# Apokleos/kata-xpu-device-plugin

Hardware: AMD Instinct MI355X
Metric: Allocate() p50 latency (lower is better)
Workload: dtype n/a; 1 GPU; model=kata-xpu-device-plugin-amd pod-churn, node=8x MI355X (mock sysfs, vfio-pci), gpus_per_pod=1, discovered_gpus=8, concurrent_clients=1, parallelism=1 churn client(s), one plugin daemon

## Files before the change

kata_xpu_device_plugin_amd/plugin/manager.py:

```python
from __future__ import annotations

import os
import signal
import threading
from typing import Dict, List, Optional

from ..cdi.spec import build_spec, write_spec
from ..config import Config
from ..discovery.naming import resource_name
from ..discovery.sysfs import NodeInventory, XPUDevice, scan_node
from ..health.watcher import NodeWatcher
from ..topology.hive import GPUTopology, load_topology
from ..utils.log import configure as configure_logging, get_logger
from .server import XPUDevicePlugin
from .state import DeviceState

log = get_logger(__name__)


class PluginManager:
    def __init__(self, cfg: Config):
        cfg.validate()
        self.cfg = cfg
        self.inventory: Optional[NodeInventory] = None
        self.topology: Optional[GPUTopology] = None
        self.plugins: Dict[str, XPUDevicePlugin] = {}
        self.states: Dict[str, DeviceState] = {}
        self.watcher: Optional[NodeWatcher] = None
        self.cdi_spec_path: Optional[str] = None
        self._stop = threading.Event()
        self._register = True
        self._rescan_lock = threading.Lock()
        self._metrics = None
        self._amdsmi = None
        self._gpu_probe = None
        self._rescan_thread = None

    def _group_by_resource(self, inv: NodeInventory) -> Dict[str, Dict[str, XPUDevice]]:
        out: Dict[str, Dict[str, XPUDevice]] = {}
        for gid, dev in inv.devices.items():
            rname = resource_name(
                dev.model_device_id,
                namespace=self.cfg.resource_namespace,
                pci_ids_paths=tuple(self.cfg.pci_ids_paths),
                is_vf=dev.is_vf,
                unified=self.cfg.unified_resource_name,
            )
            out.setdefault(rname, {})[gid] = dev
        return out

    def _write_cdi(self, inv: NodeInventory) -> Optional[str]:
        if not inv.devices:
            from ..cdi.spec import spec_path
            for fmt in ("yaml", "json"):
                stale = spec_path(self.cfg.cdi_dir, self.cfg.cdi_spec_name, fmt)
                if os.path.exists(stale):
                    try:
                        os.unlink(stale)
                    except OSError:
                        pass
            log.info("no devices: no CDI spec written")
            return None
        spec = build_spec(inv, self.cfg.cdi_kind, self.cfg.dev_root,
                          self.cfg.cdi_version)
        return write_spec(
            spec, self.cfg.cdi_dir, self.cfg.cdi_spec_name, self.cfg.cdi_format
        )

    def setup(self) -> None:
        inv = scan_node(self.cfg)
        self.inventory = inv
        log.info(
            "discovered %d xPU device(s) in %.1f ms (%d %s function(s) total)",
            len(inv.devices), inv.scan_wall_s * 1e3, len(inv.all_functions),
            "/".join(f"{v:04x}" for v in self.cfg.vendor_allowlist),
        )
        self.topology = load_topology(self.cfg, inv)
        log.info("xGMI topology source: %s (%d hive-mapped GPUs)",
                 self.topology.source, len(self.topology.hive_of))

        self.cdi_spec_path = self._write_cdi(inv)

        for rname, devs in sorted(self._group_by_resource(inv).items()):
            state = DeviceState(devs)
            self.states[rname] = state
            self.plugins[rname] = XPUDevicePlugin(
                self.cfg, rname, state, self.topology
            )
            log.info("resource %s: %d device(s): %s", rname, len(devs),
                     ",".join(sorted(devs)))

    def start(self, register: bool = True) -> None:
        self._register = register
        if not self.plugins:
            log.warning("no devices discovered; serving nothing (will still "
                        "watch for kubelet restarts)")
        for plugin in self.plugins.values():
            plugin.start(register=register)
        self.watcher = NodeWatcher(
            self.cfg,
            self.states,
            on_socket_removed=self._on_socket_removed,
            on_kubelet_restarted=self._on_kubelet_restarted,
            plugin_socket_names={p.socket_name for p in self.plugins.values()},
            on_cdi_spec_removed=self._on_cdi_spec_removed,
            cdi_spec_names={os.path.basename(self.cdi_spec_path)}
            if self.cdi_spec_path else set(),
        )
        self.watcher.start()
        self.watcher.wait_ready()
        if self.cfg.amdsmi_health:
            from ..health.amdsmi_health import AmdSmiPoller
            self._amdsmi = AmdSmiPoller(
                self.cfg.health_poll_interval_s, self._on_amdsmi_health,
                on_xgmi=self._on_xgmi_telemetry,
            )
            self._amdsmi.start()
        if self.cfg.gpu_probe_interval_s > 0:
            from ..health.probe_poller import GpuProbePoller
            self._gpu_probe = GpuProbePoller(
                self.cfg.gpu_probe_interval_s, self._on_probe_health
            )
            self._gpu_probe.start()
        if self.cfg.rescan_interval_s > 0:
            self._rescan_thread = threading.Thread(
                target=self._rescan_loop, name="kxdp-rescan", daemon=True)
            self._rescan_thread.start()
        if self.cfg.metrics_port:
            from ..metrics import MetricsExporter
            self._metrics = MetricsExporter(self)
            self._metrics.start(self.cfg.metrics_port)
        if self.cfg.gc_tuning:
            self._tune_gc()
        if self.cfg.cpu_affinity:
            self._pin_cpus(self.cfg.cpu_affinity)

    @staticmethod
    def _pin_cpus(spec: str) -> None:
        cpus = set()
        try:
            for part in spec.split(","):
                part = part.strip()
                if not part:
                    continue
                if "-" in part:
                    lo, hi = part.split("-", 1)
                    cpus.update(range(int(lo), int(hi) + 1))
                else:
                    cpus.add(int(part))
            if cpus:
                os.sched_setaffinity(0, cpus)
                log.info("pinned daemon to CPUs %s", sorted(cpus))
        except (ValueError, OSError) as e:
            log.warning("cpu_affinity %r not applied: %s", spec, e)

    @staticmethod
    def _tune_gc() -> None:
        import gc
        gc.collect()
        gc.freeze()
        gc.set_threshold(50_000, 20, 20)

    def _on_socket_removed(self, socket_name: str) -> None:
        for plugin in list(self.plugins.values()):
            if plugin.socket_name == socket_name and not self._stop.is_set():
                if plugin.consume_expected_removal():
                    log.info("socket removal of %s was self-inflicted; skipping", socket_name)
                    continue
                if os.path.exists(plugin.socket_path) and plugin.serving:
                    continue
                try:
                    log.warning("EXTERNAL socket removal; restarting %s", plugin.resource_name)
                    plugin.restart()
                except Exception:
                    log.exception("restart of %s failed", plugin.resource_name)

    def _on_cdi_spec_removed(self, name: str) -> None:
        if self._stop.is_set() or self.inventory is None:
            return
        try:
            self.cdi_spec_path = self._write_cdi(self.inventory)
        except Exception:
            log.exception("CDI spec regeneration failed")

    def _on_amdsmi_health(self, bdf: str, healthy: bool, reasons) -> None:
        for state in list(self.states.values()):
            for gid in state.device_ids():
                dev = state.device(gid)
                if dev and bdf in (fn.bdf.lower() for fn in dev.functions):
                    if not healthy:
                        log.warning("amd-smi: %s unhealthy: %s", bdf, reasons)
                    state.set_health(gid, healthy, source="amdsmi")
                    return

    def _on_xgmi_telemetry(self, snap) -> None:
        if self.topology is None:
            return
        sick = {bdf for bdf, dh in snap.items() if dh.xgmi_sick}
        if sick != set(self.topology.degraded):
            if sick:
                log.warning("xGMI degraded link(s) on %s — excluded from "
                            "hive placement", sorted(sick))
            else:
                log.info("xGMI links recovered; hive placement restored")
            self.topology.set_degraded(sick)

    def _rescan_loop(self) -> None:
        while not self._stop.wait(self.cfg.rescan_interval_s):
            try:
                self.rescan()
            except Exception:
                log.exception("periodic rescan failed")

    def _on_probe_health(self, bdf: str, healthy: bool) -> None:
        bdf = bdf.lower()
        for state in list(self.states.values()):
            for gid in state.device_ids():
                dev = state.device(gid)
                if dev and bdf in (fn.bdf.lower() for fn in dev.functions):
                    if not healthy:
                        log.warning("gpu probe: %s unhealthy", bdf)
                    state.set_health(gid, healthy, source="probe")
                    return

    def _on_kubelet_restarted(self) -> None:
        if self._stop.is_set():
            return
        for plugin in list(self.plugins.values()):
            try:
                plugin.register_with_kubelet()
            except Exception:
                log.exception("re-registration of %s failed", plugin.resource_name)

    def install_signal_handlers(self) -> None:
        def _sig(signum, frame):
            log.info("signal %d — shutting down", signum)
            self._stop.set()

        def _hup(signum, frame):
            log.info("SIGHUP — rescanning inventory")
            threading.Thread(target=self._safe_rescan, name="kxdp-hup-rescan",
                             daemon=True).start()

        signal.signal(signal.SIGTERM, _sig)
        signal.signal(signal.SIGINT, _sig)
        signal.signal(signal.SIGHUP, _hup)

    def _safe_rescan(self) -> None:
        try:
            if not self._stop.is_set():
                self.rescan()
        except Exception:
            log.exception("SIGHUP rescan failed")

    def run_forever(self) -> None:
        self.install_signal_handlers()
        self._stop.wait()
        self.stop()

    def stop(self) -> None:
        self._stop.set()
        if self.watcher is not None:
            self.watcher.stop()
            self.watcher = None
        if self._amdsmi is not None:
            self._amdsmi.stop()
            self._amdsmi = None
        if self._gpu_probe is not None:
            self._gpu_probe.stop()
            self._gpu_probe = None
        for plugin in list(self.plugins.values()):
            plugin.stop()
        if self._metrics is not None:
            self._metrics.stop()
            self._metrics = None

    @staticmethod
    def _inventory_signature(inv: NodeInventory):
        return {
            gid: (tuple(dev.bdfs), dev.model_device_id, dev.numa_node,
                  dev.is_vf)
            for gid, dev in inv.devices.items()
        }

    def rescan(self) -> bool:
        with self._rescan_lock:
            return self._rescan_locked()

    def _rescan_locked(self) -> bool:
        inv = scan_node(self.cfg)
        if self.inventory is not None and \
                self._inventory_signature(inv) == \
                self._inventory_signature(self.inventory):
            return False
        log.info("rescan: inventory changed (%d → %d devices)",
                 len(self.inventory.devices) if self.inventory else 0,
                 len(inv.devices))
        self.inventory = inv
        prev_degraded = self.topology.degraded if self.topology else frozenset()
        self.topology = load_topology(self.cfg, inv)
        self.topology.degraded = prev_degraded
        self.cdi_spec_path = self._write_cdi(inv)
        grouped = self._group_by_resource(inv)

        for rname, state in list(self.states.items()):
            if rname in grouped:
                state.replace_devices(grouped[rname])
                self.plugins[rname].topo = self.topology

        retiring = [r for r in self.plugins if r not in grouped]
        if retiring and self.watcher is not None:
            self.watcher.plugin_socket_names = {
                p.socket_name for r, p in self.plugins.items()
                if r not in retiring}
        for rname in retiring:
            plugin = self.plugins.pop(rname)
            self.states.pop(rname, None)
            try:
                plugin.stop()
            except Exception:
                log.exception("stopping retired plugin %s failed", rname)
            log.info("resource %s retired (no devices after rescan)", rname)

        for rname in sorted(set(grouped) - set(self.plugins)):
            state = DeviceState(grouped[rname])
            plugin = XPUDevicePlugin(self.cfg, rname, state, self.topology)
            self.states[rname] = state
            self.plugins[rname] = plugin
            if self.watcher is not None:
                try:
                    plugin.start(register=self._register)
                    log.info("resource %s: started dynamically (%d devices)",
                             rname, len(grouped[rname]))
                except Exception:
                    log.exception("dynamic start of %s failed", rname)

        if self.watcher is not None:
            self.watcher.plugin_socket_names = {
                p.socket_name for p in self.plugins.values()}
        return True


def main(argv: Optional[List[str]] = None) -> int:
    import argparse

    parser = argparse.ArgumentParser(
        prog="kata-xpu-device-plugin-amd",
        description="MI355X-native Kubernetes device plugin for VFIO/Kata GPU passthrough",
    )
    Config.add_args(parser)
    args = parser.parse_args(argv)
    cfg = Config.from_args(args)
    configure_logging(cfg.log_level)
    mgr = PluginManager(cfg)
    mgr.install_signal_handlers()
    mgr.setup()
    mgr.start()
    mgr.run_forever()
    return 0


if __name__ == "__main__":
    raise SystemExit(main())
```

kata_xpu_device_plugin_amd/plugin/server.py:

```python
from __future__ import annotations

import asyncio
import atexit
import os
import threading
import time
import weakref
from typing import Dict, List, Optional

import grpc
import grpc.aio

from ..cdi.spec import ANNOTATION_PREFIX, qualified_name
from ..config import Config, STRATEGY_CDI_ANNOTATIONS, STRATEGY_CDI_CRI
from ..discovery.sysfs import read_hex, read_link_base
from ..topology.hive import GPUTopology, preferred_sets
from ..utils.log import get_logger
from . import api
from .state import DeviceState

log = get_logger(__name__)

try:
    from .. import _native as _NATIVE
except ImportError:
    _NATIVE = None

ENV_CDI_VENDOR_CLASS = "KUBERNETES_CDI_VENDOR_CLASS"
ENV_PCI_RESOURCE_PREFIX = "PCI_RESOURCE_"

_DEVICE_PLUGIN_PATH = "/v1beta1.DevicePlugin/"

_LIVE_NATIVE = weakref.WeakSet()


@atexit.register
def _stop_native_servers() -> None:
    for plugin in list(_LIVE_NATIVE):
        srv = plugin._native_server
        if srv is not None:
            try:
                srv.stop(0.0)
            except Exception:
                pass


def _stream_open() -> None:
    """DeviceState subscription of one open native ListAndWatch stream."""


def native_server_available() -> bool:
    return _NATIVE is not None and hasattr(_NATIVE, "GrpcServer")


class AllocationError(Exception):
    pass


class XPUDevicePlugin:

    def __init__(
        self,
        cfg: Config,
        resource_name: str,
        state: DeviceState,
        topo: GPUTopology,
        socket_name: Optional[str] = None,
    ):
        self.cfg = cfg
        self.resource_name = resource_name
        self.state = state
        self.topo = topo
        short = resource_name.split("/", 1)[1].lower()
        self.socket_name = socket_name or f"{cfg.plugin_socket_prefix}-{short}.sock"
        self.socket_path = os.path.join(cfg.kubelet_socket_dir, self.socket_name)
        self._aio_server: Optional[grpc.aio.Server] = None
        self._loop: Optional[asyncio.AbstractEventLoop] = None
        self._thread: Optional[threading.Thread] = None
        self._stop = threading.Event()
        self._serving = threading.Event()
        self._lifecycle = threading.Lock()
        self._removal_lock = threading.Lock()
        self._expected_removals = 0
        self.watcher_servicer = None
        self.watcher_socket_path: Optional[str] = None
        self._allocations = 0
        self._allocate_failures = 0
        self._last_allocate_s = 0.0
        self._allocate_seconds_total = 0.0
        self._native_server = None
        self._native_unsubscribe = None
        self._stream_subscriptions: List = []
        self._devices_dir = os.path.join(cfg.sysfs_root, "bus", "pci", "devices")
        self._vendor_list = list(cfg.vendor_allowlist)
        self._qn_cache: Dict[str, str] = {}
        self._bdf_cache = None
        self._timing = {"allocate_us": [], "preferred_us": [],
                        "loop_lag_us": []} if cfg.rpc_timing_path else None
        self._env_res_name = ENV_PCI_RESOURCE_PREFIX + resource_name.upper(
        ).replace("/", "_").replace(".", "_").replace("-", "_")

    def _native_stats(self):
        srv = self._native_server
        return srv.stats() if srv is not None else (0, 0, None, 0.0)

    @property
    def allocations(self) -> int:
        return self._allocations + self._native_stats()[0]

    @allocations.setter
    def allocations(self, v: int) -> None:
        self._allocations = v

    @property
    def allocate_failures(self) -> int:
        return self._allocate_failures + self._native_stats()[1]

    @allocate_failures.setter
    def allocate_failures(self, v: int) -> None:
        self._allocate_failures = v

    @property
    def last_allocate_s(self) -> float:
        last = self._native_stats()[2]
        return self._last_allocate_s if not last else last

    @last_allocate_s.setter
    def last_allocate_s(self, v: float) -> None:
        self._last_allocate_s = v

    @property
    def allocate_seconds_total(self) -> float:
        return self._allocate_seconds_total + self._native_stats()[3]

    @allocate_seconds_total.setter
    def allocate_seconds_total(self, v: float) -> None:
        self._allocate_seconds_total = v

    def _qn(self, gid: str) -> str:
        qn = self._qn_cache.get(gid)
        if qn is None:
            qn = self._qn_cache[gid] = qualified_name(self.cfg.cdi_kind, gid)
        return qn

    async def GetDevicePluginOptions(self, request, context):
        return api.DevicePluginOptions(
            pre_start_required=False,
            get_preferred_allocation_available=True,
        )

    def _device_list(self, snapshot=None) -> List[object]:
        devs = []
        if snapshot is None:
            snapshot = self.state.snapshot()
        for dev, healthy in snapshot:
            d = api.Device(
                id=dev.id,
                health=api.HEALTHY if healthy else api.UNHEALTHY,
            )
            if dev.numa_node >= 0:
                d.topology.nodes.add(id=dev.numa_node)
            devs.append(d)
        return devs

    async def ListAndWatch(self, request, context):
        loop = asyncio.get_running_loop()
        event = asyncio.Event()

        def _notify() -> None:
            try:
                loop.call_soon_threadsafe(event.set)
            except RuntimeError:
                pass

        unsubscribe = self.state.subscribe(_notify)
        try:
            yield api.ListAndWatchResponse(devices=self._device_list())
            while not self._stop.is_set():
                await event.wait()
                event.clear()
                if self._stop.is_set():
                    break
                yield api.ListAndWatchResponse(devices=self._device_list())
        finally:
            unsubscribe()

    def _revalidate_many(self, ids: List[str]) -> None:
        groups = []
        for gid in ids:
            dev = self.state.device(gid)
            if dev is None:
                raise AllocationError(f"unknown device id {gid}")
            if self.cfg.reject_unhealthy and not self.state.is_healthy(gid):
                raise AllocationError(f"device {gid} is Unhealthy")
            groups.append((gid, [fn.bdf for fn in dev.functions]))
        if self.cfg.native != "off":
            if _NATIVE is None and self.cfg.native == "require":
                raise RuntimeError("_native extension required but missing")
            if _NATIVE is not None:
                err = _NATIVE.revalidate_groups(
                    self._devices_dir, groups,
                    self._vendor_list, self.cfg.required_driver,
                )
                if err:
                    raise AllocationError(err)
                return
        for gid, _bdfs in groups:
            self._revalidate_py(gid)

    def _revalidate_py(self, gid: str) -> None:
        dev = self.state.device(gid)
        assert dev is not None
        devices_dir = self._devices_dir
        for fn in dev.functions:
            p = os.path.join(devices_dir, fn.bdf)
            if read_link_base(os.path.join(p, "iommu_group")) != gid:
                raise AllocationError(f"device {fn.bdf} no longer in IOMMU group {gid}")
            vendor = read_hex(os.path.join(p, "vendor"))
            if vendor not in set(self.cfg.vendor_allowlist):
                raise AllocationError(f"device {fn.bdf} vendor {vendor:#x} not allowed")
            if read_link_base(os.path.join(p, "driver")) != self.cfg.required_driver:
                raise AllocationError(
                    f"device {fn.bdf} not bound to {self.cfg.required_driver}"
                )

    def _container_response(self, ids: List[str]):
        resp = api.ContainerAllocateResponse()
        strategy = self.cfg.device_list_strategy
        bdfs: List[str] = []
        if ids and strategy not in (STRATEGY_CDI_CRI, STRATEGY_CDI_ANNOTATIONS):
            vfio_ctl = os.path.join(self.cfg.dev_root, "vfio", "vfio")
            resp.devices.add(
                container_path=vfio_ctl, host_path=vfio_ctl, permissions="rw"
            )
        for gid in ids:
            dev = self.state.device(gid)
            assert dev is not None
            bdfs.extend(dev.bdfs)
            if strategy == STRATEGY_CDI_CRI:
                resp.cdi_devices.add(name=self._qn(gid))
            elif strategy == STRATEGY_CDI_ANNOTATIONS:
                key = f"{ANNOTATION_PREFIX}vfio{gid}"
                resp.annotations[key] = self._qn(gid)
            else:
                path = os.path.join(self.cfg.dev_root, dev.vfio_node)
                resp.devices.add(
                    container_path=path, host_path=path, permissions="rw"
                )
        if strategy in (STRATEGY_CDI_CRI, STRATEGY_CDI_ANNOTATIONS):
            resp.envs[ENV_CDI_VENDOR_CLASS] = self.cfg.cdi_kind
        resp.envs[self._env_res_name] = ",".join(bdfs)
        return resp

    async def Allocate(self, request, context):
        t0 = time.perf_counter()
        response = api.AllocateResponse()
        try:
            for creq in request.container_requests:
                ids = list(creq.devices_ids)
                self._revalidate_many(ids)
                response.container_responses.append(self._container_response(ids))
        except AllocationError as e:
            self.allocate_failures += 1
            log.warning("Allocate(%s) rejected: %s", self.resource_name, e)
            await context.abort(grpc.StatusCode.INVALID_ARGUMENT, str(e))
        self.allocations += 1
        self.last_allocate_s = time.perf_counter() - t0
        self.allocate_seconds_total += self.last_allocate_s
        if self._timing is not None:
            self._timing["allocate_us"].append(self.last_allocate_s * 1e6)
        return response

    async def GetPreferredAllocation(self, request, context):
        return self._preferred_allocation(request)

    def _preferred_allocation(self, request):
        t0 = time.perf_counter() if self._timing is not None else 0.0
        resp = api.PreferredAllocationResponse()
        gen = self.state.generation
        cached = self._bdf_cache
        if cached is not None and cached[0] == gen:
            bdf_of = cached[1]
        else:
            bdf_of = self.state.bdf_map()
            self._bdf_cache = (gen, bdf_of)
        for creq in request.container_requests:
            available = [d for d in creq.available_device_ids if d in bdf_of]
            must = list(creq.must_include_device_ids)
            pick = preferred_sets(
                self.topo, bdf_of, available, must, creq.allocation_size
            )
            resp.container_responses.add(device_ids=pick)
        if self._timing is not None:
            self._timing["preferred_us"].append(
                (time.perf_counter() - t0) * 1e6)
        return resp

    async def PreStartContainer(self, request, context):
        return api.PreStartContainerResponse()

    def start(self, register: bool = True) -> None:
        with self._lifecycle:
            self._start_locked(register)

    def _use_native_server(self) -> bool:
        want = self.cfg.grpc_server
        if want == "aio":
            return False
        if native_server_available() and self.cfg.native != "off":
            return True
        if want == "native":
            raise RuntimeError(
                "grpc_server=native needs the _native extension "
                "(and native != off)")
        if self.cfg.native == "require":
            raise RuntimeError("_native extension required but missing")
        return False

    def _start_locked(self, register: bool) -> None:
        self._stop.clear()
        if self._use_native_server():
            self._start_native()
        else:
            self._start_aio()
        ch = grpc.insecure_channel(f"unix://{self.socket_path}")
        try:
            grpc.channel_ready_future(ch).result(timeout=self.cfg.grpc_timeout_s)
        finally:
            ch.close()
        self._serving.set()
        if register and self.cfg.registration_mode in ("legacy", "both"):
            try:
                self.register_with_kubelet()
            except Exception as e:
                log.warning("kubelet registration failed (%s); serving "
                            "anyway and retrying in background", e)
                self._spawn_registration_retry()
        log.info("plugin %s serving on %s (%s registration)",
                 self.resource_name, self.socket_path,
                 self.cfg.registration_mode)

    def _start_aio(self) -> None:
        self._loop_ready = threading.Event()
        self._start_error: Optional[BaseException] = None
        self._thread = threading.Thread(
            target=self._serve_thread,
            name=f"kxdp-grpc-{self.resource_name.split('/')[-1]}",
            daemon=True,
        )
        self._thread.start()
        if not self._loop_ready.wait(self.cfg.grpc_timeout_s):
            raise RuntimeError(f"gRPC server for {self.resource_name} "
                               "did not start in time")
        if self._start_error is not None:
            self._thread.join(timeout=2.0)
            raise self._start_error

    def _start_native(self) -> None:
        os.makedirs(self.cfg.kubelet_socket_dir, exist_ok=True)
        if os.path.exists(self.socket_path):
            self._note_expected_removal()
            os.unlink(self.socket_path)
        paths = [self.socket_path]
        if self.cfg.registration_mode in ("watcher", "both"):
            from .watcher_registration import (
                SERVICE_PATH_PREFIX,
                WatcherRegistrationServicer,
            )
            os.makedirs(self.cfg.plugins_registry_dir, exist_ok=True)
            self.watcher_servicer = WatcherRegistrationServicer(
                self.resource_name, self.socket_path)
            self.watcher_socket_path = os.path.join(
                self.cfg.plugins_registry_dir, self.socket_name)
            if os.path.exists(self.watcher_socket_path):
                os.unlink(self.watcher_socket_path)
            paths.append(self.watcher_socket_path)
        srv = _NATIVE.GrpcServer(paths)
        p = _DEVICE_PLUGIN_PATH
        srv.register_constant(
            p + "GetDevicePluginOptions",
            api.DevicePluginOptions(
                pre_start_required=False,
                get_preferred_allocation_available=True,
            ).SerializeToString())
        srv.register_constant(
            p + "PreStartContainer",
            api.PreStartContainerResponse().SerializeToString())
        srv.register_watch(p + "ListAndWatch", self._on_watch_streams)
        srv.register_unary(p + "GetPreferredAllocation",
                           self._preferred_allocation_bytes)
        srv.configure_allocate(
            p + "Allocate",
            strategy=self.cfg.device_list_strategy,
            reject_unhealthy=bool(self.cfg.reject_unhealthy),
            cdi_kind=self.cfg.cdi_kind,
            env_name=self._env_res_name,
            dev_root=self.cfg.dev_root,
            devices_dir=self._devices_dir,
            vendors=self._vendor_list,
            required_driver=self.cfg.required_driver,
            on_reject=self._log_rejection,
            timing=self._timing is not None,
        )
        if self.watcher_servicer is not None and len(paths) > 1:
            srv.register_unary(SERVICE_PATH_PREFIX + "GetInfo",
                               self.watcher_servicer.get_info_bytes)
            srv.register_unary(
                SERVICE_PATH_PREFIX + "NotifyRegistrationStatus",
                self.watcher_servicer.notify_registration_status_bytes)
        self._native_server = srv
        self._native_unsubscribe = self.state.subscribe_snapshot(
            self._push_native_state)
        try:
            srv.start()
        except BaseException:
            self._native_unsubscribe()
            self._native_unsubscribe = None
            self._native_server = None
            raise
        _LIVE_NATIVE.add(self)

    def _push_native_state(self, snapshot, generation) -> None:
        srv = self._native_server
        if srv is None:
            return
        dev_root = self.cfg.dev_root
        rows = []
        for dev, healthy in snapshot:
            qn = self._qn(dev.id)
            rows.append((
                dev.id,
                [fn.bdf for fn in dev.functions],
                bool(healthy),
                api.CDIDevice(name=qn).SerializeToString(),
                f"{ANNOTATION_PREFIX}vfio{dev.id}",
                qn,
                os.path.join(dev_root, dev.vfio_node),
            ))
        srv.update_table(rows)
        srv.publish(api.ListAndWatchResponse(
            devices=self._device_list(snapshot)).SerializeToString())

    def _on_watch_streams(self, delta: int) -> None:
        subs = self._stream_subscriptions
        for _ in range(delta):
            subs.append(self.state.subscribe(_stream_open))
        for _ in range(-delta):
            if subs:
                subs.pop()()

    def _preferred_allocation_bytes(self, request: bytes) -> bytes:
        return self._preferred_allocation(
            api.PreferredAllocationRequest.FromString(request)
        ).SerializeToString()

    def _log_rejection(self, err: str) -> None:
        log.warning("Allocate(%s) rejected: %s", self.resource_name, err)

    def _stop_native(self) -> None:
        srv = self._native_server
        if srv is None:
            return
        if self._native_unsubscribe is not None:
            self._native_unsubscribe()
            self._native_unsubscribe = None
        srv.stop(1.0)
        n, fails, last, total = srv.stats()
        if self._timing is not None:
            self._timing["allocate_us"] = list(srv.allocate_timing_us())
            self._timing["loop_lag_us"] = []
            self._dump_timing()
        self._native_server = None
        _LIVE_NATIVE.discard(self)
        while self._stream_subscriptions:
            self._stream_subscriptions.pop()()
        self._allocations += n
        self._allocate_failures += fails
        self._allocate_seconds_total += total
        if last:
            self._last_allocate_s = last

    def _spawn_registration_retry(self) -> None:
        def retry():
            delay = 1.0
            while self._serving.is_set() and not self._stop.is_set():
                if self._stop.wait(delay):
                    return
                if not self._serving.is_set():
                    return
                try:
                    self.register_with_kubelet()
                    log.info("kubelet registration succeeded after retry")
                    return
                except Exception:
                    delay = min(delay * 2, 30.0)

        threading.Thread(target=retry, daemon=True,
                         name=f"kxdp-register-retry-{self.socket_name}").start()

    def _serve_thread(self) -> None:
        loop = asyncio.new_event_loop()
        self._loop = loop
        asyncio.set_event_loop(loop)

        async def _main():
            server = grpc.aio.server(
                options=[("grpc.max_concurrent_streams", 64),
                         ("grpc.optimization_target", "latency")])
            api.add_device_plugin_servicer(server, self)
            os.makedirs(self.cfg.kubelet_socket_dir, exist_ok=True)
            if os.path.exists(self.socket_path):
                self._note_expected_removal()
                os.unlink(self.socket_path)
            server.add_insecure_port(f"unix://{self.socket_path}")
            if self.cfg.registration_mode in ("watcher", "both"):
                from .watcher_registration import (
                    WatcherRegistrationServicer,
                    add_watcher_registration_servicer,
                )
                os.makedirs(self.cfg.plugins_registry_dir, exist_ok=True)
                self.watcher_servicer = WatcherRegistrationServicer(
                    self.resource_name, self.socket_path)
                self.watcher_socket_path = os.path.join(
                    self.cfg.plugins_registry_dir, self.socket_name)
                add_watcher_registration_servicer(server, self.watcher_servicer)
                if os.path.exists(self.watcher_socket_path):
                    os.unlink(self.watcher_socket_path)
                server.add_insecure_port(f"unix://{self.watcher_socket_path}")
            await server.start()
            self._aio_server = server
            self._stop_async = asyncio.Event()
            lag_task = None
            if self._timing is not None:
                async def _lag_monitor():
                    while not self._stop_async.is_set():
                        t0 = time.perf_counter()
                        await asyncio.sleep(0.001)
                        lag = (time.perf_counter() - t0 - 0.001) * 1e6
                        self._timing["loop_lag_us"].append(max(0.0, lag))
                        if len(self._timing["loop_lag_us"]) > 200_000:
                            del self._timing["loop_lag_us"][:100_000]
                lag_task = asyncio.ensure_future(_lag_monitor())
            self._loop_ready.set()
            await self._stop_async.wait()
            if lag_task is not None:
                lag_task.cancel()
            await server.stop(grace=1.0)
            if self._timing is not None:
                self._dump_timing()

        try:
            loop.run_until_complete(_main())
        except BaseException as e:
            self._start_error = e
            self._loop_ready.set()
        finally:
            try:
                loop.close()
            except Exception:
                pass

    def _dump_timing(self) -> None:
        import json
        import statistics as stats

        def dist(xs):
            if not xs:
                return None
            xs = sorted(xs)
            n = len(xs)
            return {"n": n,
                    "p50": round(xs[n // 2], 1),
                    "p90": round(xs[min(n - 1, int(n * 0.9))], 1),
                    "p99": round(xs[min(n - 1, int(n * 0.99))], 1),
                    "max": round(xs[-1], 1),
                    "mean": round(stats.fmean(xs), 1)}

        out = {k: dist(v) for k, v in self._timing.items()}
        path = f"{self.cfg.rpc_timing_path}.{self.socket_name}.json"
        try:
            with open(path, "w") as f:
                json.dump(out, f, indent=1)
            log.info("rpc timing breakdown → %s", path)
        except OSError as e:
            log.warning("could not write rpc timing: %s", e)

    def register_with_kubelet(self) -> None:
        ch = grpc.insecure_channel(f"unix://{self.cfg.kubelet_socket}")
        try:
            grpc.channel_ready_future(ch).result(timeout=self.cfg.grpc_timeout_s)
            stub = api.RegistrationStub(ch)
            stub.Register(
                api.RegisterRequest(
                    version=api.VERSION,
                    endpoint=self.socket_name,
                    resource_name=self.resource_name,
                    options=api.DevicePluginOptions(
                        pre_start_required=False,
                        get_preferred_allocation_available=True,
                    ),
                ),
                timeout=self.cfg.grpc_timeout_s,
            )
        finally:
            ch.close()

    def stop(self) -> None:
        with self._lifecycle:
            self._stop_locked()

    def _stop_locked(self) -> None:
        self._stop.set()
        self._serving.clear()
        self.state.poke()
        if os.path.exists(self.socket_path):
            self._note_expected_removal()
        self._stop_native()
        if self._loop is not None and getattr(self, "_stop_async", None) is not None:
            try:
                self._loop.call_soon_threadsafe(self._stop_async.set)
            except RuntimeError:
                pass
        if self._thread is not None:
            self._thread.join(timeout=5.0)
            self._thread = None
        self._aio_server = None
        self._loop = None
        for path in (self.socket_path,
                     getattr(self, "watcher_socket_path", None)):
            if path and os.path.exists(path):
                try:
                    os.unlink(path)
                except OSError:
                    pass

    def restart(self, register: bool = True) -> None:
        self.stop()
        self.start(register=register)

    def _note_expected_removal(self) -> None:
        with self._removal_lock:
            self._expected_removals += 1

    def consume_expected_removal(self) -> bool:
        with self._removal_lock:
            if self._expected_removals > 0:
                self._expected_removals -= 1
                return True
            return False

    @property
    def serving(self) -> bool:
        return self._serving.is_set()
```

kata_xpu_device_plugin_amd/plugin/state.py:

```python
from __future__ import annotations

import queue
import threading
from typing import Callable, Dict, List, Optional, Tuple

from ..discovery.sysfs import XPUDevice
from ..utils.log import get_logger

log = get_logger(__name__)


class DeviceState:

    def __init__(self, devices: Dict[str, XPUDevice]):
        self._lock = threading.Lock()
        self._devices: Dict[str, XPUDevice] = dict(devices)
        self._unhealthy_by: Dict[str, set] = {gid: set() for gid in devices}
        self._watchers: List[queue.Queue] = []
        self._callbacks: List[Callable[[], None]] = []
        self._snapshot_callbacks: List[Callable[[list, int], None]] = []
        self._generation = 0

    def _snapshot_locked(self) -> List[Tuple[XPUDevice, bool]]:
        return [(self._devices[g], not self._unhealthy_by[g])
                for g in sorted(self._devices, key=_gkey)]

    def snapshot(self) -> List[Tuple[XPUDevice, bool]]:
        with self._lock:
            return self._snapshot_locked()

    def device(self, gid: str) -> Optional[XPUDevice]:
        with self._lock:
            return self._devices.get(gid)

    def device_ids(self) -> List[str]:
        with self._lock:
            return sorted(self._devices, key=_gkey)

    def healthy_ids(self) -> List[str]:
        with self._lock:
            return sorted((g for g, u in self._unhealthy_by.items() if not u),
                          key=_gkey)

    def is_healthy(self, gid: str) -> bool:
        with self._lock:
            u = self._unhealthy_by.get(gid)
            return u is not None and not u

    @property
    def generation(self) -> int:
        with self._lock:
            return self._generation

    def bdf_map(self) -> Dict[str, str]:
        with self._lock:
            return {gid: dev.primary.bdf for gid, dev in self._devices.items()}

    def set_health(self, gid: str, healthy: bool, source: str = "vfio") -> bool:
        with self._lock:
            if gid not in self._devices:
                return False
            u = self._unhealthy_by[gid]
            before = not u
            if healthy:
                u.discard(source)
            else:
                u.add(source)
            after = not u
            if before == after:
                return False
            self._generation += 1
            self._notify_locked()
        log.info("device %s → %s (source %s)", gid,
                 "Healthy" if after else "Unhealthy", source)
        return True

    def replace_devices(self, devices: Dict[str, XPUDevice]) -> None:
        with self._lock:
            old = self._unhealthy_by
            self._devices = dict(devices)
            self._unhealthy_by = {g: set(old.get(g, set())) for g in devices}
            self._generation += 1
            self._notify_locked()

    def _notify_locked(self, changed: bool = True) -> None:
        if changed and self._snapshot_callbacks:
            snap = self._snapshot_locked()
            for scb in self._snapshot_callbacks:
                try:
                    scb(snap, self._generation)
                except Exception:
                    log.exception("state snapshot subscriber failed")
        for q in self._watchers:
            try:
                q.put_nowait(self._generation)
            except queue.Full:
                pass
        for cb in self._callbacks:
            try:
                cb()
            except Exception:
                pass

    def watch(self) -> queue.Queue:
        q: queue.Queue = queue.Queue(maxsize=64)
        with self._lock:
            self._watchers.append(q)
        return q

    def unwatch(self, q: queue.Queue) -> None:
        with self._lock:
            try:
                self._watchers.remove(q)
            except ValueError:
                pass

    def subscribe(self, cb: Callable[[], None]) -> Callable[[], None]:
        with self._lock:
            self._callbacks.append(cb)

        def unsubscribe() -> None:
            with self._lock:
                try:
                    self._callbacks.remove(cb)
                except ValueError:
                    pass
        return unsubscribe

    def subscribe_snapshot(
        self, cb: Callable[[List[Tuple[XPUDevice, bool]], int], None],
    ) -> Callable[[], None]:
        with self._lock:
            self._snapshot_callbacks.append(cb)
            cb(self._snapshot_locked(), self._generation)

        def unsubscribe() -> None:
            with self._lock:
                try:
                    self._snapshot_callbacks.remove(cb)
                except ValueError:
                    pass
        return unsubscribe

    def poke(self) -> None:
        with self._lock:
            self._notify_locked(changed=False)


def _gkey(g: str):
    return (0, int(g)) if g.isdigit() else (1, g)
```

native/pbwire.h:

```cpp
#pragma once

#include <cstddef>
#include <cstdint>
#include <string>
#include <vector>

namespace kxdp {
namespace pb {

inline void put_varint(std::string& out, uint64_t v) {
    while (v >= 128) {
        out.push_back((char)((v & 0x7f) | 0x80));
        v >>= 7;
    }
    out.push_back((char)v);
}

inline void put_bytes(std::string& out, uint32_t field, const char* p, size_t n) {
    put_varint(out, ((uint64_t)field << 3) | 2);
    put_varint(out, n);
    out.append(p, n);
}

inline void put_bytes(std::string& out, uint32_t field, const std::string& s) {
    put_bytes(out, field, s.data(), s.size());
}

inline void put_map_entry(std::string& out, uint32_t field,
                          const std::string& key, const std::string& value) {
    std::string e;
    put_bytes(e, 1, key);
    put_bytes(e, 2, value);
    put_bytes(out, field, e);
}

struct Reader {
    const uint8_t* p;
    const uint8_t* end;

    Reader(const void* data, size_t n)
        : p((const uint8_t*)data), end((const uint8_t*)data + n) {}

    bool done() const { return p >= end; }

    bool varint(uint64_t& v) {
        v = 0;
        for (int shift = 0; shift < 64; shift += 7) {
            if (p >= end) return false;
            uint8_t b = *p++;
            v |= (uint64_t)(b & 0x7f) << shift;
            if (!(b & 0x80)) return true;
        }
        return false;
    }

    bool tag(uint32_t& field, uint32_t& wire) {
        uint64_t t;
        if (!varint(t) || (t >> 3) == 0 || (t >> 3) > 0x1fffffff) return false;
        field = (uint32_t)(t >> 3);
        wire = (uint32_t)(t & 7);
        return true;
    }

    bool bytes(const uint8_t*& data, size_t& n) {
        uint64_t len;
        if (!varint(len) || len > (uint64_t)(end - p)) return false;
        data = p;
        n = (size_t)len;
        p += len;
        return true;
    }

    bool skip(uint32_t wire) {
        uint64_t v;
        const uint8_t* d;
        size_t n;
        switch (wire) {
        case 0: return varint(v);
        case 1: if (end - p < 8) return false; p += 8; return true;
        case 2: return bytes(d, n);
        case 5: if (end - p < 4) return false; p += 4; return true;
        default: return false;
        }
    }
};

inline bool parse_allocate_request(
    const std::string& msg, std::vector<std::vector<std::string>>& out) {
    Reader r(msg.data(), msg.size());
    while (!r.done()) {
        uint32_t field, wire;
        if (!r.tag(field, wire)) return false;
        if (field == 1 && wire == 2) {
            const uint8_t* d;
            size_t n;
            if (!r.bytes(d, n)) return false;
            out.emplace_back();
            Reader c(d, n);
            while (!c.done()) {
                uint32_t cf, cw;
                if (!c.tag(cf, cw)) return false;
                if (cf == 1 && cw == 2) {
                    const uint8_t* s;
                    size_t sn;
                    if (!c.bytes(s, sn)) return false;
                    out.back().emplace_back((const char*)s, sn);
                } else if (!c.skip(cw)) {
                    return false;
                }
            }
        } else if (!r.skip(wire)) {
            return false;
        }
    }
    return true;
}

}
}
```

native/xpu_grpc_server.cpp:

```cpp
#include <pybind11/pybind11.h>
#include <pybind11/stl.h>

#include <atomic>
#include <cerrno>
#include <chrono>
#include <cstring>
#include <fcntl.h>
#include <memory>
#include <mutex>
#include <poll.h>
#include <stdexcept>
#include <sys/epoll.h>
#include <sys/eventfd.h>
#include <sys/socket.h>
#include <sys/uio.h>
#include <sys/un.h>
#include <thread>
#include <unistd.h>
#include <unordered_map>

#include "h2.h"
#include "pbwire.h"

namespace py = pybind11;
using namespace kxdp;

namespace {

constexpr int STRATEGY_CDI_CRI = 0;
constexpr int STRATEGY_CDI_ANNOTATIONS = 1;
constexpr int STRATEGY_DEVICE_NODES = 2;
constexpr size_t kMaxTimingSamples = 1u << 20;

struct DeviceEntry {
    std::vector<std::string> bdfs;
    bool healthy = true;
    std::string cdi_device;
    std::string ann_key, ann_value;
    std::string dev_path;
};

using Table = std::unordered_map<std::string, DeviceEntry>;

struct AllocateConfig {
    bool enabled = false;
    std::string path;
    int strategy = STRATEGY_CDI_CRI;
    bool reject_unhealthy = true;
    std::string cdi_kind, env_name, dev_root, devices_dir, required_driver;
    std::vector<long> vendors;
    bool timing = false;
};

enum class Kind { CONSTANT, WATCH, PYTHON, ALLOCATE };

struct Method {
    Kind kind;
    std::string bytes;
    py::object fn;
};

std::string link_base(int dirfd, const char* name) {
    char buf[512];
    ssize_t n = ::readlinkat(dirfd, name, buf, sizeof(buf) - 1);
    if (n <= 0) return {};
    buf[n] = 0;
    const char* slash = std::strrchr(buf, '/');
    return std::string(slash ? slash + 1 : buf);
}

long read_vendor(int dirfd) {
    int fd = ::openat(dirfd, "vendor", O_RDONLY | O_CLOEXEC);
    if (fd < 0) return -1;
    char buf[64];
    ssize_t n = ::read(fd, buf, sizeof(buf) - 1);
    ::close(fd);
    if (n <= 0) return -1;
    buf[n] = 0;
    errno = 0;
    char* end = nullptr;
    long v = std::strtol(buf, &end, 16);
    if (errno || end == buf) return -1;
    return v;
}

struct IoConn {
    int fd;
    h2::Conn h2;
    size_t woff = 0;
    size_t watching = 0;
    bool want_write = false;
    IoConn(int f, h2::App* app) : fd(f), h2(app) {}
};

class GrpcServer : public h2::App {
public:
    explicit GrpcServer(std::vector<std::string> paths)
        : paths_(std::move(paths)) {}

    ~GrpcServer() override {
        if (thread_.joinable()) {
            py::gil_scoped_release rel;
            request_stop(0.0);
            thread_.join();
        }
        methods_.clear();
        on_reject_ = py::object();
        on_watch_change_ = py::object();
    }

    void register_constant(const std::string& path, const std::string& bytes) {
        check_not_running();
        methods_[path] = Method{Kind::CONSTANT, bytes, py::object()};
    }
    void register_watch(const std::string& path, py::object on_change) {
        check_not_running();
        methods_[path] = Method{Kind::WATCH, {}, py::object()};
        on_watch_change_ = std::move(on_change);
    }
    void register_unary(const std::string& path, py::object fn) {
        check_not_running();
        methods_[path] = Method{Kind::PYTHON, {}, std::move(fn)};
    }
    void configure_allocate(const std::string& path, const std::string& strategy,
                            bool reject_unhealthy, const std::string& cdi_kind,
                            const std::string& env_name,
                            const std::string& dev_root,
                            const std::string& devices_dir,
                            const std::vector<long>& vendors,
                            const std::string& required_driver,
                            py::object on_reject, bool timing) {
        check_not_running();
        alloc_.enabled = true;
        alloc_.path = path;
        alloc_.strategy = strategy == "cdi-cri" ? STRATEGY_CDI_CRI
                          : strategy == "cdi-annotations" ? STRATEGY_CDI_ANNOTATIONS
                          : STRATEGY_DEVICE_NODES;
        alloc_.reject_unhealthy = reject_unhealthy;
        alloc_.cdi_kind = cdi_kind;
        alloc_.env_name = env_name;
        alloc_.dev_root = dev_root;
        alloc_.devices_dir = devices_dir;
        alloc_.vendors = vendors;
        alloc_.required_driver = required_driver;
        alloc_.timing = timing;
        on_reject_ = std::move(on_reject);
        methods_[path] = Method{Kind::ALLOCATE, {}, py::object()};
    }

    void update_table(const std::vector<std::tuple<
            std::string, std::vector<std::string>, bool, py::bytes,
            std::string, std::string, std::string>>& devices) {
        auto t = std::make_shared<Table>();
        for (auto& d : devices) {
            DeviceEntry e;
            e.bdfs = std::get<1>(d);
            e.healthy = std::get<2>(d);
            e.cdi_device = std::string(std::get<3>(d));
            e.ann_key = std::get<4>(d);
            e.ann_value = std::get<5>(d);
            e.dev_path = std::get<6>(d);
            (*t)[std::get<0>(d)] = std::move(e);
        }
        std::lock_guard<std::mutex> g(table_mu_);
        table_ = std::move(t);
    }

    void publish(const std::string& message) {
        auto m = std::make_shared<const std::string>(message);
        {
            std::lock_guard<std::mutex> g(pub_mu_);
            latest_ = std::move(m);
            pub_gen_++;
        }
        wake();
    }

    void start() {
        if (thread_.joinable()) throw std::runtime_error("server already started");
        stop_.store(false);
        ep_ = ::epoll_create1(EPOLL_CLOEXEC);
        wake_fd_ = ::eventfd(0, EFD_NONBLOCK | EFD_CLOEXEC);
        if (ep_ < 0 || wake_fd_ < 0) {
            close_fds();
            throw std::runtime_error("epoll/eventfd setup failed");
        }
        add_epoll(wake_fd_, EPOLLIN);
        for (auto& path : paths_) {
            sockaddr_un addr{};
            addr.sun_family = AF_UNIX;
            if (path.size() >= sizeof(addr.sun_path)) {
                close_fds();
                throw std::runtime_error("socket path too long: " + path);
            }
            std::memcpy(addr.sun_path, path.c_str(), path.size() + 1);
            int fd = ::socket(AF_UNIX, SOCK_STREAM | SOCK_NONBLOCK | SOCK_CLOEXEC, 0);
            if (fd < 0 || ::bind(fd, (sockaddr*)&addr, sizeof(addr)) < 0 ||
                ::listen(fd, 128) < 0) {
                std::string why = std::strerror(errno);
                if (fd >= 0) ::close(fd);
                close_fds();
                throw std::runtime_error("cannot listen on " + path + ": " + why);
            }
            listeners_.push_back(fd);
            bound_.push_back(path);
            add_epoll(fd, EPOLLIN);
        }
        thread_ = std::thread([this] { run(); });
    }

    void stop(double grace) {
        if (!thread_.joinable()) return;
        py::gil_scoped_release rel;
        request_stop(grace);
        thread_.join();
    }

    bool running() const { return thread_.joinable(); }

    py::tuple stats() {
        std::lock_guard<std::mutex> g(stat_mu_);
        return py::make_tuple(allocations_, failures_, last_s_, total_s_);
    }

    std::vector<double> allocate_timing_us() {
        std::lock_guard<std::mutex> g(stat_mu_);
        return alloc_us_;
    }

    void on_rpc(h2::Conn& c, uint32_t sid, const std::string& path,
                std::string& msg) override {
        auto it = methods_.find(path);
        if (it == methods_.end())
            return c.reply_error(sid, h2::GRPC_UNIMPLEMENTED, "Method not found!");
        Method& m = it->second;
        switch (m.kind) {
        case Kind::CONSTANT:
            return c.reply_unary(sid, m.bytes);
        case Kind::ALLOCATE:
            return handle_allocate(c, sid, msg);
        case Kind::WATCH: {
            std::shared_ptr<const std::string> latest;
            {
                std::lock_guard<std::mutex> g(pub_mu_);
                latest = latest_;
            }
            c.start_stream(sid);
            if (latest) c.push_message(sid, *latest);
            return;
        }
        case Kind::PYTHON:
            return handle_python(c, sid, m, msg);
        }
    }

private:
    void check_not_running() {
        if (thread_.joinable())
            throw std::runtime_error("register methods before start()");
    }

    void wake() {
        if (wake_fd_ >= 0) {
            uint64_t one = 1;
            ssize_t r = ::write(wake_fd_, &one, sizeof(one));
            (void)r;
        }
    }

    void request_stop(double grace) {
        grace_s_ = grace;
        stop_.store(true);
        wake();
    }

    void add_epoll(int fd, uint32_t events) {
        epoll_event ev{};
        ev.events = events;
        ev.data.fd = fd;
        ::epoll_ctl(ep_, EPOLL_CTL_ADD, fd, &ev);
    }

    void close_fds() {
        for (int fd : listeners_) ::close(fd);
        listeners_.clear();
        for (auto& p : bound_) ::unlink(p.c_str());
        bound_.clear();
        if (wake_fd_ >= 0) ::close(wake_fd_);
        if (ep_ >= 0) ::close(ep_);
        wake_fd_ = ep_ = -1;
        if (dirfd_ >= 0) ::close(dirfd_);
        dirfd_ = -1;
        dirfd_table_ = nullptr;
    }

    struct GilHold {
        PyThreadState*& ts;
        bool held = false;
        explicit GilHold(PyThreadState*& t) : ts(t) {
            if (ts && !_Py_IsFinalizing()) {
                PyEval_RestoreThread(ts);
                held = true;
            }
        }
        ~GilHold() {
            if (held) ts = PyEval_SaveThread();
        }
    };

    void handle_python(h2::Conn& c, uint32_t sid, Method& m, std::string& msg) {
        bool ok = false;
        int status = h2::GRPC_UNKNOWN;
        std::string payload;
        {
            GilHold gil(ts_);
            if (!gil.held) {
                status = h2::GRPC_UNAVAILABLE;
                payload = "server shutting down";
            } else {
                try {
                    py::object r = m.fn(py::bytes(msg));
                    if (py::isinstance<py::bytes>(r)) {
                        payload = r.cast<std::string>();
                        ok = true;
                    } else {
                        auto t = r.cast<std::pair<int, std::string>>();
                        status = t.first;
                        payload = t.second;
                    }
                } catch (py::error_already_set& e) {
                    try {
                        payload = "Unexpected " +
                                  py::str(e.type()).cast<std::string>() + ": " +
                                  py::str(e.value()).cast<std::string>();
                    } catch (...) {
                        payload = "handler raised";
                    }
                    e.restore();
                    PyErr_Clear();
                } catch (std::exception& e) {
                    payload = e.what();
                }
            }
        }
        if (ok) c.reply_unary(sid, payload);
        else c.reply_error(sid, status, payload);
    }

    void report_watchers(IoConn& io, size_t now) {
        if (now == io.watching) return;
        long delta = (long)now - (long)io.watching;
        io.watching = now;
        GilHold gil(ts_);
        if (!gil.held || !on_watch_change_ || on_watch_change_.is_none()) return;
        try {
            on_watch_change_(delta);
        } catch (py::error_already_set& e) {
            e.restore();
            PyErr_Clear();
        }
    }

    void log_rejection(const std::string& err) {
        GilHold gil(ts_);
        if (!gil.held || !on_reject_ || on_reject_.is_none()) return;
        try {
            on_reject_(err);
        } catch (py::error_already_set& e) {
            e.restore();
            PyErr_Clear();
        }
    }

    bool open_devices_dir() {
        if (dirfd_ >= 0) ::close(dirfd_);
        dirfd_ = ::open(alloc_.devices_dir.c_str(),
                        O_RDONLY | O_DIRECTORY | O_CLOEXEC);
        return dirfd_ >= 0;
    }

    std::string revalidate(const std::string& gid, const DeviceEntry& dev) {
        for (const auto& bdf : dev.bdfs) {
            const int flags = O_RDONLY | O_DIRECTORY | O_CLOEXEC;
            int dfd = ::openat(dirfd_, bdf.c_str(), flags);
            if (dfd < 0) {
                if (!open_devices_dir())
                    return "cannot open " + alloc_.devices_dir;
                dfd = ::openat(dirfd_, bdf.c_str(), flags);
            }
            if (dfd < 0) return "device " + bdf + " vanished";
            std::string err;
            if (link_base(dfd, "iommu_group") != gid) {
                err = "device " + bdf + " no longer in IOMMU group " + gid;
            } else {
                long vendor = read_vendor(dfd);
                if (vendor < 0 ||
                    std::find(alloc_.vendors.begin(), alloc_.vendors.end(),
                              vendor) == alloc_.vendors.end())
                    err = "device " + bdf + " vendor not allowed";
                else if (link_base(dfd, "driver") != alloc_.required_driver)
                    err = "device " + bdf + " not bound to " +
                          alloc_.required_driver;
            }
            ::close(dfd);
            if (!err.empty()) return err;
        }
        return {};
    }

    std::string allocate_container(const Table& table,
                                   const std::vector<std::string>& ids,
                                   std::string& out) {
        std::vector<const DeviceEntry*> devs;
        devs.reserve(ids.size());
        for (const auto& gid : ids) {
            auto it = table.find(gid);
            if (it == table.end()) return "unknown device id " + gid;
            if (alloc_.reject_unhealthy && !it->second.healthy)
                return "device " + gid + " is Unhealthy";
            devs.push_back(&it->second);
        }
        if (dirfd_ < 0 || dirfd_table_ != &table) {
            if (!open_devices_dir()) return "cannot open " + alloc_.devices_dir;
            dirfd_table_ = &table;
        }
        for (size_t i = 0; i < ids.size(); i++) {
            std::string err = revalidate(ids[i], *devs[i]);
            if (!err.empty()) return err;
        }
        const bool cdi = alloc_.strategy != STRATEGY_DEVICE_NODES;
        std::string bdfs;
        for (auto* d : devs)
            for (const auto& b : d->bdfs) {
                if (!bdfs.empty()) bdfs.push_back(',');
                bdfs += b;
            }
        static const std::string kVendorClass = "KUBERNETES_CDI_VENDOR_CLASS";
        if (cdi && alloc_.env_name == kVendorClass) {
            pb::put_map_entry(out, 1, alloc_.env_name, bdfs);
        } else if (cdi && kVendorClass < alloc_.env_name) {
            pb::put_map_entry(out, 1, kVendorClass, alloc_.cdi_kind);
            pb::put_map_entry(out, 1, alloc_.env_name, bdfs);
        } else {
            pb::put_map_entry(out, 1, alloc_.env_name, bdfs);
            if (cdi) pb::put_map_entry(out, 1, kVendorClass, alloc_.cdi_kind);
        }
        if (!cdi) {
            auto spec = [&](const std::string& path) {
                std::string s;
                pb::put_bytes(s, 1, path);
                pb::put_bytes(s, 2, path);
                pb::put_bytes(s, 3, "rw", 2);
                pb::put_bytes(out, 3, s);
            };
            if (!ids.empty()) spec(alloc_.dev_root + "/vfio/vfio");
            for (auto* d : devs) spec(d->dev_path);
        }
        if (alloc_.strategy == STRATEGY_CDI_ANNOTATIONS)
            for (auto* d : devs)
                pb::put_map_entry(out, 4, d->ann_key, d->ann_value);
        if (alloc_.strategy == STRATEGY_CDI_CRI)
            for (auto* d : devs) pb::put_bytes(out, 5, d->cdi_device);
        return {};
    }

    void handle_allocate(h2::Conn& c, uint32_t sid, const std::string& msg) {
        auto t0 = std::chrono::steady_clock::now();
        std::shared_ptr<const Table> table;
        {
            std::lock_guard<std::mutex> g(table_mu_);
            table = table_;
        }
        std::vector<std::vector<std::string>> reqs;
        if (!pb::parse_allocate_request(msg, reqs))
            return c.reply_error(sid, h2::GRPC_INTERNAL,
                                 "Exception deserializing request!");
        static const Table kEmpty;
        const Table& tbl = table ? *table : kEmpty;
        std::string resp, err;
        for (const auto& ids : reqs) {
            std::string cresp;
            err = allocate_container(tbl, ids, cresp);
            if (!err.empty()) break;
            pb::put_bytes(resp, 1, cresp);
        }
        if (!err.empty()) {
            {
                std::lock_guard<std::mutex> g(stat_mu_);
                failures_++;
            }
            c.reply_error(sid, h2::GRPC_INVALID_ARGUMENT, err);
            log_rejection(err);
            return;
        }
        double dt = std::chrono::duration<double>(
                        std::chrono::steady_clock::now() - t0).count();
        {
            std::lock_guard<std::mutex> g(stat_mu_);
            allocations_++;
            last_s_ = dt;
            total_s_ += dt;
            if (alloc_.timing && alloc_us_.size() < kMaxTimingSamples)
                alloc_us_.push_back(dt * 1e6);
        }
        c.reply_unary(sid, resp);
    }

    void set_want_write(IoConn& io, bool on) {
        if (io.want_write == on) return;
        io.want_write = on;
        epoll_event ev{};
        ev.events = EPOLLIN | (on ? EPOLLOUT : 0);
        ev.data.fd = io.fd;
        ::epoll_ctl(ep_, EPOLL_CTL_MOD, io.fd, &ev);
    }

    bool flush(IoConn& io) {
        std::string& out = io.h2.out();
        while (io.woff < out.size()) {
            iovec iov{(void*)(out.data() + io.woff), out.size() - io.woff};
            msghdr mh{};
            mh.msg_iov = &iov;
            mh.msg_iovlen = 1;
            ssize_t n = ::sendmsg(io.fd, &mh, MSG_NOSIGNAL);
            if (n < 0) {
                if (errno == EINTR) continue;
                if (errno == EAGAIN || errno == EWOULDBLOCK) {
                    set_want_write(io, true);
                    return true;
                }
                return false;
            }
            io.woff += (size_t)n;
        }
        out.clear();
        io.woff = 0;
        set_want_write(io, false);
        return !io.h2.want_close();
    }

    void close_conn(int fd) {
        auto it = conns_.find(fd);
        if (it == conns_.end()) return;
        report_watchers(*it->second, 0);
        ::epoll_ctl(ep_, EPOLL_CTL_DEL, fd, nullptr);
        ::close(fd);
        conns_.erase(it);
    }

    void on_readable(IoConn& io) {
        ssize_t n = ::read(io.fd, rbuf_, sizeof(rbuf_));
        if (n == 0) return close_conn(io.fd);
        if (n < 0) {
            if (errno == EAGAIN || errno == EINTR) return;
            return close_conn(io.fd);
        }
        io.h2.feed((const uint8_t*)rbuf_, (size_t)n);
        report_watchers(io, io.h2.watch_streams());
        if (!flush(io)) close_conn(io.fd);
    }

    void deliver_publications() {
        std::shared_ptr<const std::string> latest;
        uint64_t gen;
        {
            std::lock_guard<std::mutex> g(pub_mu_);
            latest = latest_;
            gen = pub_gen_;
        }
        if (gen == pub_seen_ || !latest) return;
        pub_seen_ = gen;
        std::vector<int> done;
        for (auto& kv : conns_) {
            kv.second->h2.broadcast(*latest);
            if (!flush(*kv.second)) done.push_back(kv.first);
        }
        for (int fd : done) close_conn(fd);
    }

    void shutdown_connections() {
        for (int fd : listeners_) ::close(fd);
        listeners_.clear();
        for (auto& p : bound_) ::unlink(p.c_str());
        bound_.clear();
        for (auto& kv : conns_) kv.second->h2.begin_shutdown();
        auto deadline = std::chrono::steady_clock::now() +
                        std::chrono::duration<double>(grace_s_);
        for (auto& kv : conns_) {
            IoConn& io = *kv.second;
            while (flush(io) && io.woff < io.h2.out().size()) {
                auto left = std::chrono::duration_cast<std::chrono::milliseconds>(
                    deadline - std::chrono::steady_clock::now()).count();
                if (left <= 0) break;
                pollfd p{io.fd, POLLOUT, 0};
                if (::poll(&p, 1, (int)left) <= 0) break;
            }
            ::shutdown(io.fd, SHUT_WR);
            while (::read(io.fd, rbuf_, sizeof(rbuf_)) > 0) {}
            report_watchers(io, 0);
            ::close(io.fd);
        }
        conns_.clear();
    }

    void run() {
        PyGILState_STATE gstate = PyGILState_Ensure();
        ts_ = PyEval_SaveThread();
        epoll_event evs[64];
        while (!stop_.load()) {
            int n = ::epoll_wait(ep_, evs, 64, -1);
            if (n < 0) {
                if (errno == EINTR) continue;
                break;
            }
            for (int i = 0; i < n && !stop_.load(); i++) {
                int fd = evs[i].data.fd;
                if (fd == wake_fd_) {
                    uint64_t v;
                    while (::read(wake_fd_, &v, sizeof(v)) > 0) {}
                    deliver_publications();
                    continue;
                }
                if (std::find(listeners_.begin(), listeners_.end(), fd) !=
                    listeners_.end()) {
                    for (;;) {
                        int cfd = ::accept4(fd, nullptr, nullptr,
                                            SOCK_NONBLOCK | SOCK_CLOEXEC);
                        if (cfd < 0) break;
                        auto io = std::make_unique<IoConn>(cfd, this);
                        IoConn& ref = *io;
                        conns_[cfd] = std::move(io);
                        add_epoll(cfd, EPOLLIN);
                        if (!flush(ref)) close_conn(cfd);
                    }
                    continue;
                }
                auto it = conns_.find(fd);
                if (it == conns_.end()) continue;
                IoConn& io = *it->second;
                if (evs[i].events & EPOLLOUT) {
                    if (!flush(io)) {
                        close_conn(fd);
                        continue;
                    }
                }
                if (evs[i].events & (EPOLLIN | EPOLLHUP | EPOLLERR))
                    on_readable(io);
            }
        }
        shutdown_connections();
        if (!_Py_IsFinalizing()) {
            PyEval_RestoreThread(ts_);
            PyGILState_Release(gstate);
        }
        ts_ = nullptr;
        int ep = ep_, wfd = wake_fd_;
        ep_ = wake_fd_ = -1;
        ::close(ep);
        ::close(wfd);
        if (dirfd_ >= 0) ::close(dirfd_);
        dirfd_ = -1;
        dirfd_table_ = nullptr;
    }

    std::vector<std::string> paths_, bound_;
    std::unordered_map<std::string, Method> methods_;
    AllocateConfig alloc_;
    py::object on_reject_, on_watch_change_;

    std::mutex table_mu_;
    std::shared_ptr<const Table> table_;
    std::mutex pub_mu_;
    std::shared_ptr<const std::string> latest_;
    uint64_t pub_gen_ = 0;
    uint64_t pub_seen_ = 0;

    std::mutex stat_mu_;
    uint64_t allocations_ = 0, failures_ = 0;
    double last_s_ = 0.0, total_s_ = 0.0;
    std::vector<double> alloc_us_;

    std::thread thread_;
    std::atomic<bool> stop_{false};
    double grace_s_ = 1.0;
    int ep_ = -1, wake_fd_ = -1;
    std::vector<int> listeners_;
    std::unordered_map<int, std::unique_ptr<IoConn>> conns_;
    PyThreadState* ts_ = nullptr;
    int dirfd_ = -1;
    const Table* dirfd_table_ = nullptr;
    char rbuf_[65536];
};

}

void kxdp_init_grpc_server(py::module_& m) {
    py::class_<GrpcServer>(m, "GrpcServer")
        .def(py::init<std::vector<std::string>>(), py::arg("socket_paths"))
        .def("register_constant", &GrpcServer::register_constant,
             py::arg("path"), py::arg("response"))
        .def("register_watch", &GrpcServer::register_watch, py::arg("path"),
             py::arg("on_change") = py::none())
        .def("register_unary", &GrpcServer::register_unary, py::arg("path"),
             py::arg("fn"),
             "fn(request bytes) -> response bytes | (status code, message)")
        .def("configure_allocate", &GrpcServer::configure_allocate,
             py::arg("path"), py::arg("strategy"), py::arg("reject_unhealthy"),
             py::arg("cdi_kind"), py::arg("env_name"), py::arg("dev_root"),
             py::arg("devices_dir"), py::arg("vendors"),
             py::arg("required_driver"), py::arg("on_reject"),
             py::arg("timing") = false)
        .def("update_table", &GrpcServer::update_table, py::arg("devices"))
        .def("publish", &GrpcServer::publish, py::arg("message"))
        .def("start", &GrpcServer::start)
        .def("stop", &GrpcServer::stop, py::arg("grace") = 1.0)
        .def("stats", &GrpcServer::stats)
        .def("allocate_timing_us", &GrpcServer::allocate_timing_us)
        .def_property_readonly("running", &GrpcServer::running);
}
```

native/xpu_native.cpp:

```cpp

#include <pybind11/pybind11.h>
#include <pybind11/stl.h>

#include <algorithm>
#include <cstdint>
#include <cstring>
#include <dirent.h>
#include <functional>
#include <fcntl.h>
#include <map>
#include <optional>
#include <string>
#include <unistd.h>
#include <vector>

namespace py = pybind11;

namespace {

static std::string read_attr(int dirfd, const char* name) {
    int fd = ::openat(dirfd, name, O_RDONLY | O_CLOEXEC);
    if (fd < 0) return {};
    char buf[256];
    ssize_t n = ::read(fd, buf, sizeof(buf) - 1);
    ::close(fd);
    if (n <= 0) return {};
    buf[n] = 0;
    while (n > 0 && (buf[n - 1] == '\n' || buf[n - 1] == ' ')) buf[--n] = 0;
    return std::string(buf, (size_t)n);
}

static std::optional<long> parse_hex(const std::string& s) {
    if (s.empty()) return std::nullopt;
    errno = 0;
    char* end = nullptr;
    long v = std::strtol(s.c_str(), &end, 16);
    if (errno || end == s.c_str()) return std::nullopt;
    return v;
}

static std::optional<long> parse_int(const std::string& s) {
    if (s.empty()) return std::nullopt;
    errno = 0;
    char* end = nullptr;
    long v = std::strtol(s.c_str(), &end, 10);
    if (errno || end == s.c_str()) return std::nullopt;
    return v;
}

static std::string link_base(int dirfd, const char* name) {
    char buf[512];
    ssize_t n = ::readlinkat(dirfd, name, buf, sizeof(buf) - 1);
    if (n <= 0) return {};
    buf[n] = 0;
    const char* slash = std::strrchr(buf, '/');
    return std::string(slash ? slash + 1 : buf);
}

struct Fn {
    std::string bdf;
    long vendor = 0, device = 0, class_code = 0;
    std::string driver, iommu_group, physfn;
    long numa = -1, totalvfs = 0, numvfs = 0;
};

static std::optional<Fn> read_function(int base_fd, const std::string& bdf,
                                       const std::vector<long>& vendors) {
    int dfd = ::openat(base_fd, bdf.c_str(), O_RDONLY | O_DIRECTORY | O_CLOEXEC);
    if (dfd < 0) return std::nullopt;
    Fn fn;
    fn.bdf = bdf;
    auto vendor = parse_hex(read_attr(dfd, "vendor"));
    if (!vendor ||
        std::find(vendors.begin(), vendors.end(), *vendor) == vendors.end()) {
        ::close(dfd);
        return std::nullopt;
    }
    fn.vendor = *vendor;
    auto device = parse_hex(read_attr(dfd, "device"));
    if (!device) { ::close(dfd); return std::nullopt; }
    fn.device = *device;
    fn.class_code = parse_hex(read_attr(dfd, "class")).value_or(0);
    fn.driver = link_base(dfd, "driver");
    fn.iommu_group = link_base(dfd, "iommu_group");
    fn.physfn = link_base(dfd, "physfn");
    fn.numa = parse_int(read_attr(dfd, "numa_node")).value_or(-1);
    fn.totalvfs = parse_int(read_attr(dfd, "sriov_totalvfs")).value_or(0);
    fn.numvfs = parse_int(read_attr(dfd, "sriov_numvfs")).value_or(0);
    ::close(dfd);
    return fn;
}

py::list scan_pci(const std::string& devices_dir, const std::vector<long>& vendors) {
    py::list out;
    int base_fd = ::open(devices_dir.c_str(), O_RDONLY | O_DIRECTORY | O_CLOEXEC);
    if (base_fd < 0) return out;
    std::vector<std::string> names;
    {
        DIR* d = ::fdopendir(::dup(base_fd));
        if (d) {
            while (dirent* ent = ::readdir(d)) {
                if (ent->d_name[0] == '.') continue;
                names.emplace_back(ent->d_name);
            }
            ::closedir(d);
        }
    }
    std::sort(names.begin(), names.end());
    for (const auto& bdf : names) {
        auto fn = read_function(base_fd, bdf, vendors);
        if (!fn) continue;
        py::dict d;
        d["bdf"] = fn->bdf;
        d["vendor"] = fn->vendor;
        d["device"] = fn->device;
        d["class_code"] = fn->class_code;
        d["driver"] = fn->driver.empty() ? py::object(py::none())
                                         : py::object(py::str(fn->driver));
        d["iommu_group"] = fn->iommu_group.empty()
                               ? py::object(py::none())
                               : py::object(py::str(fn->iommu_group));
        d["numa_node"] = fn->numa;
        d["sriov_totalvfs"] = fn->totalvfs;
        d["sriov_numvfs"] = fn->numvfs;
        d["physfn_bdf"] = fn->physfn.empty() ? py::object(py::none())
                                             : py::object(py::str(fn->physfn));
        out.append(std::move(d));
    }
    ::close(base_fd);
    return out;
}

std::string revalidate_group(const std::string& devices_dir,
                             const std::string& group_id,
                             const std::vector<std::string>& bdfs,
                             const std::vector<long>& vendors,
                             const std::string& required_driver) {
    int base_fd = ::open(devices_dir.c_str(), O_RDONLY | O_DIRECTORY | O_CLOEXEC);
    if (base_fd < 0) return "cannot open " + devices_dir;
    std::string err;
    for (const auto& bdf : bdfs) {
        int dfd = ::openat(base_fd, bdf.c_str(), O_RDONLY | O_DIRECTORY | O_CLOEXEC);
        if (dfd < 0) { err = "device " + bdf + " vanished"; break; }
        if (link_base(dfd, "iommu_group") != group_id) {
            err = "device " + bdf + " no longer in IOMMU group " + group_id;
            ::close(dfd);
            break;
        }
        auto vendor = parse_hex(read_attr(dfd, "vendor"));
        if (!vendor ||
            std::find(vendors.begin(), vendors.end(), *vendor) == vendors.end()) {
            err = "device " + bdf + " vendor not allowed";
            ::close(dfd);
            break;
        }
        if (link_base(dfd, "driver") != required_driver) {
            err = "device " + bdf + " not bound to " + required_driver;
            ::close(dfd);
            break;
        }
        ::close(dfd);
    }
    ::close(base_fd);
    return err;
}

std::string revalidate_groups(
    const std::string& devices_dir,
    const std::vector<std::pair<std::string, std::vector<std::string>>>& groups,
    const std::vector<long>& vendors,
    const std::string& required_driver) {
    int base_fd = ::open(devices_dir.c_str(), O_RDONLY | O_DIRECTORY | O_CLOEXEC);
    if (base_fd < 0) return "cannot open " + devices_dir;
    std::string err;
    for (const auto& [gid, bdfs] : groups) {
        for (const auto& bdf : bdfs) {
            int dfd = ::openat(base_fd, bdf.c_str(),
                               O_RDONLY | O_DIRECTORY | O_CLOEXEC);
            if (dfd < 0) { err = "device " + bdf + " vanished"; goto done; }
            if (link_base(dfd, "iommu_group") != gid) {
                ::close(dfd);
                err = "device " + bdf + " no longer in IOMMU group " + gid;
                goto done;
            }
            auto vendor = parse_hex(read_attr(dfd, "vendor"));
            if (!vendor || std::find(vendors.begin(), vendors.end(), *vendor) ==
                               vendors.end()) {
                ::close(dfd);
                err = "device " + bdf + " vendor not allowed";
                goto done;
            }
            if (link_base(dfd, "driver") != required_driver) {
                ::close(dfd);
                err = "device " + bdf + " not bound to " + required_driver;
                goto done;
            }
            ::close(dfd);
        }
    }
done:
    ::close(base_fd);
    return err;
}


constexpr int64_t W_XGMI = 1000000000000LL;
constexpr int64_t W_NUMA = 1000000;
constexpr long MAX_SEARCH_NODES = 50000;

struct Bucket {
    std::string hive;
    long numa;
    std::vector<std::string> ids;
};

std::vector<std::string> select_preferred(
    const std::map<std::string, std::pair<std::string, long>>& locality,
    const std::vector<std::string>& available,
    const std::vector<std::string>& must_include,
    int size) {
    std::vector<std::string> avail;
    for (const auto& d : available)
        if (std::find(avail.begin(), avail.end(), d) == avail.end())
            avail.push_back(d);
    std::vector<std::string> must;
    for (const auto& d : must_include)
        if (std::find(must.begin(), must.end(), d) == must.end())
            must.push_back(d);
    if (size <= 0 || (size_t)size > avail.size()) return {};
    for (const auto& m : must)
        if (std::find(avail.begin(), avail.end(), m) == avail.end()) return {};
    if ((int)must.size() >= size)
        return std::vector<std::string>(must.begin(), must.begin() + size);

    const int need = size - (int)must.size();
    std::map<std::pair<std::string, long>, Bucket> bmap;
    for (const auto& d : avail) {
        if (std::find(must.begin(), must.end(), d) != must.end()) continue;
        auto it = locality.find(d);
        std::pair<std::string, long> key =
            it != locality.end() ? it->second : std::make_pair(std::string(), -1L);
        auto& b = bmap[key];
        b.hive = key.first;
        b.numa = key.second;
        b.ids.push_back(d);
    }
    std::vector<Bucket> buckets;
    for (auto& kv : bmap) {
        std::sort(kv.second.ids.begin(), kv.second.ids.end(),
                  [](const std::string& a, const std::string& b) {
                      return a.size() != b.size() ? a.size() < b.size() : a < b;
                  });
        buckets.push_back(std::move(kv.second));
    }
    std::sort(buckets.begin(), buckets.end(), [](const Bucket& a, const Bucket& b) {
        if (a.ids.size() != b.ids.size()) return a.ids.size() > b.ids.size();
        if (a.numa != b.numa) return a.numa < b.numa;
        return a.hive < b.hive;
    });

    const int nb = (int)buckets.size();
    std::vector<int64_t> affinity(nb, 0);
    for (int i = 0; i < nb; i++) {
        for (const auto& m : must) {
            auto it = locality.find(m);
            std::string mh = it != locality.end() ? it->second.first : "";
            long mn = it != locality.end() ? it->second.second : -1;
            if (!buckets[i].hive.empty() && mh == buckets[i].hive)
                affinity[i] += W_XGMI;
            else if (mn == buckets[i].numa && buckets[i].numa != -1)
                affinity[i] += W_NUMA;
        }
    }
    std::vector<int> caps(nb), suffix(nb + 1, 0);
    for (int i = 0; i < nb; i++) caps[i] = (int)buckets[i].ids.size();
    for (int i = nb - 1; i >= 0; i--) suffix[i] = suffix[i + 1] + caps[i];

    std::map<std::string, int> hive_span;
    for (int i = 0; i < nb; i++)
        if (!buckets[i].hive.empty()) hive_span[buckets[i].hive] += caps[i];
    std::vector<char> equiv(nb, 0);
    for (int i = 1; i < nb; i++) {
        const Bucket& a = buckets[i - 1];
        const Bucket& b = buckets[i];
        equiv[i] = !a.hive.empty() && !b.hive.empty() &&
                   caps[i] == caps[i - 1] && a.numa == b.numa &&
                   affinity[i] == affinity[i - 1] &&
                   hive_span[a.hive] == caps[i - 1] &&
                   hive_span[b.hive] == caps[i];
    }

    auto pkey = [&](int i) -> std::pair<std::string, long> {
        if (!buckets[i].hive.empty()) return {buckets[i].hive, -1};
        return {std::string("numa"), buckets[i].numa};
    };
    std::map<std::pair<std::string, long>, int> hive_free;
    for (int i = 0; i < nb; i++) hive_free[pkey(i)] += caps[i];

    std::vector<int64_t> max_aff_suffix(nb + 1, 0);
    for (int i = nb - 1; i >= 0; i--)
        max_aff_suffix[i] = std::max(max_aff_suffix[i + 1], affinity[i]);
    std::vector<std::map<std::string, int>> hive_cap_suffix(nb + 1);
    std::vector<std::map<long, int>> numa_cap_suffix(nb + 1);
    for (int i = nb - 1; i >= 0; i--) {
        hive_cap_suffix[i] = hive_cap_suffix[i + 1];
        numa_cap_suffix[i] = numa_cap_suffix[i + 1];
        if (!buckets[i].hive.empty()) hive_cap_suffix[i][buckets[i].hive] += caps[i];
        if (buckets[i].numa != -1) numa_cap_suffix[i][buckets[i].numa] += caps[i];
    }

    std::vector<int> take(nb, 0), best_take;
    int64_t best_score = -1;
    int64_t best_pack = 0;
    std::map<std::string, int> taken_hive;
    std::map<long, int> taken_numa;

    auto bucket_pair = [&](int i, int c) -> int64_t {
        int64_t w = !buckets[i].hive.empty() ? W_XGMI
                    : buckets[i].numa != -1 ? W_NUMA : 0;
        return w * c * (c - 1) / 2;
    };
    auto packing = [&]() -> int64_t {
        std::map<std::pair<std::string, long>, int> taken;
        for (int i = 0; i < nb; i++)
            if (take[i]) taken[pkey(i)] += take[i];
        int64_t p = 0;
        for (auto& kv : taken) p -= hive_free[kv.first] - kv.second;
        return p;
    };
    auto topk_ranges = [](const std::vector<std::pair<int, int>>& ranges,
                          int left) -> int64_t {
        if (ranges.empty() || left <= 0) return 0;
        int lo = 0, hi = 0;
        for (auto& r : ranges) hi = std::max(hi, r.first + r.second);
        while (lo < hi) {
            int mid = (lo + hi + 1) / 2;
            long cnt = 0;
            for (auto& r : ranges) {
                int top = r.first + r.second;
                if (top > mid) cnt += top - std::max(mid, r.first);
            }
            if (cnt >= left) lo = mid; else hi = mid - 1;
        }
        const int T = lo;
        int64_t total = 0;
        long cnt_above = 0;
        for (auto& r : ranges) {
            int top = r.first + r.second;
            int start = std::max(T + 1, r.first);
            if (top > start) {
                int64_t k = top - start;
                total += k * (start + top - 1) / 2;
                cnt_above += k;
            }
        }
        total += (int64_t)(left - cnt_above) * T;
        return total;
    };
    auto concentration_exact = [](const std::vector<int>& caps_desc,
                                  int left) -> int64_t {
        int64_t total = 0;
        for (int cap : caps_desc) {
            if (left <= 0) break;
            int64_t c = cap < left ? cap : left;
            total += c * (c - 1) / 2;
            left -= (int)c;
        }
        return total;
    };
    std::vector<std::vector<int>> hive_caps_desc(nb + 1), numa_caps_desc(nb + 1);
    for (int i = 0; i <= nb; i++) {
        for (auto& kv : hive_cap_suffix[i]) hive_caps_desc[i].push_back(kv.second);
        for (auto& kv : numa_cap_suffix[i]) numa_caps_desc[i].push_back(kv.second);
        std::sort(hive_caps_desc[i].rbegin(), hive_caps_desc[i].rend());
        std::sort(numa_caps_desc[i].rbegin(), numa_caps_desc[i].rend());
    }
    auto xgmi_upper = [&](int i, int left) -> int64_t {
        bool untouched = true;
        for (auto& kv : hive_cap_suffix[i]) {
            auto it = taken_hive.find(kv.first);
            if (it != taken_hive.end() && it->second > 0) { untouched = false; break; }
        }
        if (untouched) return concentration_exact(hive_caps_desc[i], left);
        std::vector<std::pair<int, int>> ranges;
        for (auto& kv : hive_cap_suffix[i]) {
            auto it = taken_hive.find(kv.first);
            int t = it != taken_hive.end() ? it->second : 0;
            ranges.emplace_back(t, kv.second);
        }
        return topk_ranges(ranges, left);
    };
    auto numa_upper = [&](int i, int left) -> int64_t {
        bool untouched = true;
        for (auto& kv : numa_cap_suffix[i]) {
            auto it = taken_numa.find(kv.first);
            if (it != taken_numa.end() && it->second > 0) { untouched = false; break; }
        }
        if (untouched) return concentration_exact(numa_caps_desc[i], left);
        std::vector<std::pair<int, int>> ranges;
        for (auto& kv : numa_cap_suffix[i]) {
            auto it = taken_numa.find(kv.first);
            int t = it != taken_numa.end() ? it->second : 0;
            ranges.emplace_back(t, kv.second);
        }
        return topk_ranges(ranges, left);
    };

    long nodes_visited = 0;
    std::function<void(int, int, int64_t)> dfs = [&](int i, int left, int64_t acc) {
        if (++nodes_visited > MAX_SEARCH_NODES && !best_take.empty()) return;
        if (left == 0) {
            int64_t pack = packing();
            if (best_take.empty() || acc > best_score ||
                (acc == best_score && pack > best_pack)) {
                best_score = acc;
                best_pack = pack;
                best_take = take;
            }
            return;
        }
        if (i >= nb || suffix[i] < left) return;
        if (!best_take.empty()) {
            int64_t ub = acc + W_XGMI * xgmi_upper(i, left) +
                         W_NUMA * numa_upper(i, left) +
                         max_aff_suffix[i] * left;
            if (ub < best_score || (ub == best_score && best_pack == 0)) return;
        }
        const std::string& hive = buckets[i].hive;
        const long numa = buckets[i].numa;
        int cmax = std::min(caps[i], left);
        if (equiv[i]) cmax = std::min(cmax, take[i - 1]);
        for (int c = cmax; c >= 0; c--) {
            int64_t inc = bucket_pair(i, c) + affinity[i] * c;
            if (c) {
                if (!hive.empty()) inc += W_XGMI * c * taken_hive[hive];
                if (numa != -1) inc += W_NUMA * c * taken_numa[numa];
                take[i] = c;
                if (!hive.empty()) taken_hive[hive] += c;
                if (numa != -1) taken_numa[numa] += c;
            }
            dfs(i + 1, left - c, acc + inc);
            if (c) {
                take[i] = 0;
                if (!hive.empty()) taken_hive[hive] -= c;
                if (numa != -1) taken_numa[numa] -= c;
            }
        }
    };
    dfs(0, need, 0);
    if (best_take.empty() && need > 0) return {};

    std::vector<std::string> chosen = must;
    for (int i = 0; i < nb; i++)
        for (int c = 0; c < best_take[i]; c++) chosen.push_back(buckets[i].ids[c]);
    return chosen;
}

}

void kxdp_init_grpc_server(py::module_& m);

PYBIND11_MODULE(_native, m) {
    m.doc() = "Native fast paths for kata-xpu-device-plugin-amd";
    m.def("scan_pci", &scan_pci, py::arg("devices_dir"), py::arg("vendors"),
          "Walk a PCI devices dir, return vendor-matched functions");
    m.def("revalidate_group", &revalidate_group, py::arg("devices_dir"),
          py::arg("group_id"), py::arg("bdfs"), py::arg("vendors"),
          py::arg("required_driver"),
          "Allocate-path group revalidation; empty string = OK");
    m.def("revalidate_groups", &revalidate_groups, py::arg("devices_dir"),
          py::arg("groups"), py::arg("vendors"), py::arg("required_driver"),
          "Batched group revalidation (one dirfd); empty string = OK");
    m.def("select_preferred", &select_preferred, py::arg("locality"),
          py::arg("available"), py::arg("must_include"), py::arg("size"),
          "Exact xGMI/NUMA bucket-composition preferred-set selection");
    kxdp_init_grpc_server(m);
}
```

setup.py:

```python
import os
import subprocess
import sys

import pybind11

ROOT = os.path.dirname(os.path.abspath(__file__))
PKG = "kata_xpu_device_plugin_amd"


def build_hip(arch: str = "gfx950", verbose: bool = True) -> str:
    import sysconfig

    hipcc = os.environ.get("HIPCC", "/opt/rocm/bin/hipcc")
    src = os.path.join(ROOT, "probes", "xpu_probe.hip")
    ext = sysconfig.get_config_var("EXT_SUFFIX") or ".so"
    out = os.path.join(ROOT, PKG, f"_gpuprobe{ext}")
    if os.path.exists(out) and os.path.getmtime(out) > os.path.getmtime(src):
        return out
    cmd = [
        hipcc, f"--offload-arch={arch}", "-O3", "-std=c++17",
        "-fPIC", "-shared",
        "-x", "hip", src,
        f"-I{pybind11.get_include()}",
        f"-I{sysconfig.get_paths()['include']}",
        "-o", out,
    ]
    if verbose:
        print("+", " ".join(cmd), file=sys.stderr)
    subprocess.run(cmd, check=True)
    return out


if __name__ == "__main__" or "setuptools" in sys.modules:
    from setuptools import Extension, setup

    if __name__ == "__main__":
        setup(
            name="kata-xpu-device-plugin-amd",
            version="0.1.0",
            packages=[
                PKG, f"{PKG}.discovery", f"{PKG}.topology", f"{PKG}.cdi",
                f"{PKG}.plugin", f"{PKG}.health", f"{PKG}.utils",
                f"{PKG}.testing", f"{PKG}.tools",
            ],
            package_data={PKG: ["data/pci.ids"]},
            include_package_data=True,
            entry_points={
                "console_scripts": [
                    "kata-xpu-device-plugin-amd=kata_xpu_device_plugin_amd.plugin.manager:main",
                    "kxdp-topo=kata_xpu_device_plugin_amd.tools.topo:main",
                    "kxdp-burnin=kata_xpu_device_plugin_amd.tools.burnin:main",
                    "kxdp-bind=kata_xpu_device_plugin_amd.tools.bind:main",
                    "kxdp-sriov=kata_xpu_device_plugin_amd.tools.sriov:main",
                    "kxdp-validate=kata_xpu_device_plugin_amd.tools.validate:main",
                    "kxdp-ident=kata_xpu_device_plugin_amd.tools.ident:main",
                    "kxdp-doctor=kata_xpu_device_plugin_amd.tools.doctor:main",
                    "kxdp-assignments=kata_xpu_device_plugin_amd.tools.assignments:main",
                    "kxdp-resourceslice=kata_xpu_device_plugin_amd.tools.resourceslice:main",
                    "kxdp-partition=kata_xpu_device_plugin_amd.tools.partition:main",
                ],
            },
            ext_modules=[
                Extension(
                    f"{PKG}._native",
                    sources=["native/xpu_native.cpp",
                             "native/xpu_grpc_server.cpp"],
                    depends=["native/h2.h", "native/hpack.h",
                             "native/pbwire.h"],
                    include_dirs=[pybind11.get_include(), "native"],
                    extra_compile_args=["-O2", "-std=c++17"],
                    extra_link_args=["-pthread"],
                    language="c++",
                ),
            ],
        )
```

Measured before the change: 48.82 us.

## Serve GetPreferredAllocation natively in C++ with locality table from device snapshot

Moves the GetPreferredAllocation RPC from a Python callback into the native gRPC server. The native server parses the request, runs the shared C++ selection search (now in prefer.h), and encodes the response, using hive and NUMA locality pushed into the native device table. Republishing is gated on generation so topology changes refresh the table without re-sending ListAndWatch. The metric is Allocate latency, so any benefit is indirect: it removes GIL and Python work from churn cycles that also call preferred allocation, at the cost of duplicated locality state that must stay in sync.

```diff
diff --git a/kata_xpu_device_plugin_amd/plugin/manager.py b/kata_xpu_device_plugin_amd/plugin/manager.py
--- a/kata_xpu_device_plugin_amd/plugin/manager.py
+++ b/kata_xpu_device_plugin_amd/plugin/manager.py
@@ -204,6 +204,8 @@
             else:
                 log.info("xGMI links recovered; hive placement restored")
             self.topology.set_degraded(sick)
+            for plugin in list(self.plugins.values()):
+                plugin.refresh_locality()
 
     def _rescan_loop(self) -> None:
         while not self._stop.wait(self.cfg.rescan_interval_s):
diff --git a/kata_xpu_device_plugin_amd/plugin/server.py b/kata_xpu_device_plugin_amd/plugin/server.py
--- a/kata_xpu_device_plugin_amd/plugin/server.py
+++ b/kata_xpu_device_plugin_amd/plugin/server.py
@@ -70,7 +70,7 @@
         self.cfg = cfg
         self.resource_name = resource_name
         self.state = state
-        self.topo = topo
+        self._topo = topo
         short = resource_name.split("/", 1)[1].lower()
         self.socket_name = socket_name or f"{cfg.plugin_socket_prefix}-{short}.sock"
         self.socket_path = os.path.join(cfg.kubelet_socket_dir, self.socket_name)
@@ -90,6 +90,7 @@
         self._allocate_seconds_total = 0.0
         self._native_server = None
         self._native_unsubscribe = None
+        self._published_generation: Optional[int] = None
         self._stream_subscriptions: List = []
         self._devices_dir = os.path.join(cfg.sysfs_root, "bus", "pci", "devices")
         self._vendor_list = list(cfg.vendor_allowlist)
@@ -99,6 +100,19 @@
                         "loop_lag_us": []} if cfg.rpc_timing_path else None
         self._env_res_name = ENV_PCI_RESOURCE_PREFIX + resource_name.upper(
         ).replace("/", "_").replace(".", "_").replace("-", "_")
+
+    @property
+    def topo(self) -> GPUTopology:
+        return self._topo
+
+    @topo.setter
+    def topo(self, topo: GPUTopology) -> None:
+        self._topo = topo
+        self.refresh_locality()
+
+    def refresh_locality(self) -> None:
+        if self._native_server is not None:
+            self.state.republish_snapshot()
 
     def _native_stats(self):
         srv = self._native_server
@@ -387,8 +401,8 @@
             p + "PreStartContainer",
             api.PreStartContainerResponse().SerializeToString())
         srv.register_watch(p + "ListAndWatch", self._on_watch_streams)
-        srv.register_unary(p + "GetPreferredAllocation",
-                           self._preferred_allocation_bytes)
+        srv.configure_preferred(p + "GetPreferredAllocation",
+                                timing=self._timing is not None)
         srv.configure_allocate(
             p + "Allocate",
             strategy=self.cfg.device_list_strategy,
@@ -409,6 +423,7 @@
                 SERVICE_PATH_PREFIX + "NotifyRegistrationStatus",
                 self.watcher_servicer.notify_registration_status_bytes)
         self._native_server = srv
+        self._published_generation = None
         self._native_unsubscribe = self.state.subscribe_snapshot(
             self._push_native_state)
         try:
@@ -425,9 +440,11 @@
         if srv is None:
             return
         dev_root = self.cfg.dev_root
+        topo = self._topo
         rows = []
         for dev, healthy in snapshot:
             qn = self._qn(dev.id)
+            bdf = dev.primary.bdf
             rows.append((
                 dev.id,
                 [fn.bdf for fn in dev.functions],
@@ -436,10 +453,14 @@
                 f"{ANNOTATION_PREFIX}vfio{dev.id}",
                 qn,
                 os.path.join(dev_root, dev.vfio_node),
+                topo.hive(bdf),
+                topo.numa_of.get(bdf, -1),
             ))
         srv.update_table(rows)
-        srv.publish(api.ListAndWatchResponse(
-            devices=self._device_list(snapshot)).SerializeToString())
+        if generation != self._published_generation:
+            self._published_generation = generation
+            srv.publish(api.ListAndWatchResponse(
+                devices=self._device_list(snapshot)).SerializeToString())
 
     def _on_watch_streams(self, delta: int) -> None:
         subs = self._stream_subscriptions
@@ -448,11 +469,6 @@
         for _ in range(-delta):
             if subs:
                 subs.pop()()
-
-    def _preferred_allocation_bytes(self, request: bytes) -> bytes:
-        return self._preferred_allocation(
-            api.PreferredAllocationRequest.FromString(request)
-        ).SerializeToString()
 
     def _log_rejection(self, err: str) -> None:
         log.warning("Allocate(%s) rejected: %s", self.resource_name, err)
@@ -468,6 +484,7 @@
         n, fails, last, total = srv.stats()
         if self._timing is not None:
             self._timing["allocate_us"] = list(srv.allocate_timing_us())
+            self._timing["preferred_us"] = list(srv.preferred_timing_us())
             self._timing["loop_lag_us"] = []
             self._dump_timing()
         self._native_server = None
diff --git a/kata_xpu_device_plugin_amd/plugin/state.py b/kata_xpu_device_plugin_amd/plugin/state.py
--- a/kata_xpu_device_plugin_amd/plugin/state.py
+++ b/kata_xpu_device_plugin_amd/plugin/state.py
@@ -83,6 +83,17 @@
             self._generation += 1
             self._notify_locked()
 
+    def republish_snapshot(self) -> None:
+        with self._lock:
+            if not self._snapshot_callbacks:
+                return
+            snap = self._snapshot_locked()
+            for scb in self._snapshot_callbacks:
+                try:
+                    scb(snap, self._generation)
+                except Exception:
+                    log.exception("state snapshot subscriber failed")
+
     def _notify_locked(self, changed: bool = True) -> None:
         if changed and self._snapshot_callbacks:
             snap = self._snapshot_locked()
diff --git a/native/pbwire.h b/native/pbwire.h
--- a/native/pbwire.h
+++ b/native/pbwire.h
@@ -116,5 +116,60 @@
     return true;
 }
 
+struct PreferredRequest {
+    std::vector<std::string> available, must_include;
+    int32_t size = 0;
+};
+
+inline bool parse_preferred_request(const std::string& msg,
+                                    std::vector<PreferredRequest>& out) {
+    Reader r(msg.data(), msg.size());
+    while (!r.done()) {
+        uint32_t field, wire;
+        if (!r.tag(field, wire)) return false;
+        if (field == 1 && wire == 2) {
+            const uint8_t* d;
+            size_t n;
+            if (!r.bytes(d, n)) return false;
+            out.emplace_back();
+            PreferredRequest& req = out.back();
+            Reader c(d, n);
+            while (!c.done()) {
+                uint32_t cf, cw;
+                if (!c.tag(cf, cw)) return false;
+                if ((cf == 1 || cf == 2) && cw == 2) {
+                    const uint8_t* s;
+                    size_t sn;
+                    if (!c.bytes(s, sn)) return false;
+                    (cf == 1 ? req.available : req.must_include)
+                        .emplace_back((const char*)s, sn);
+                } else if (cf == 3 && cw == 0) {
+                    uint64_t v;
+                    if (!c.varint(v)) return false;
+                    req.size = (int32_t)(uint32_t)v;
+                } else if (!c.skip(cw)) {
+                    return false;
+                }
+            }
+        } else if (!r.skip(wire)) {
+            return false;
+        }
+    }
+    return true;
+}
+
+inline void put_preferred_response(std::string& out,
+                                   const std::vector<std::string>& ids) {
+    size_t n = 0;
+    for (const auto& id : ids) {
+        size_t len = id.size(), lb = 1;
+        while (len >= 128) { len >>= 7; lb++; }
+        n += 1 + lb + id.size();
+    }
+    put_varint(out, (1u << 3) | 2);
+    put_varint(out, n);
+    for (const auto& id : ids) put_bytes(out, 1, id);
+}
+
 }
 }
diff --git a/native/prefer.h b/native/prefer.h
--- /dev/null
+++ b/native/prefer.h
@@ -0,0 +1,269 @@
+#pragma once
+
+#include <algorithm>
+#include <cstdint>
+#include <functional>
+#include <map>
+#include <string>
+#include <utility>
+#include <vector>
+
+namespace kxdp {
+namespace prefer {
+
+constexpr int64_t W_XGMI = 1000000000000LL;
+constexpr int64_t W_NUMA = 1000000;
+constexpr long MAX_SEARCH_NODES = 50000;
+
+using Locality = std::map<std::string, std::pair<std::string, long>>;
+
+struct Bucket {
+    std::string hive;
+    long numa;
+    std::vector<std::string> ids;
+};
+
+inline std::vector<std::string> select_preferred(
+    const Locality& locality,
+    const std::vector<std::string>& available,
+    const std::vector<std::string>& must_include,
+    int size) {
+    std::vector<std::string> avail;
+    for (const auto& d : available)
+        if (std::find(avail.begin(), avail.end(), d) == avail.end())
+            avail.push_back(d);
+    std::vector<std::string> must;
+    for (const auto& d : must_include)
+        if (std::find(must.begin(), must.end(), d) == must.end())
+            must.push_back(d);
+    if (size <= 0 || (size_t)size > avail.size()) return {};
+    for (const auto& m : must)
+        if (std::find(avail.begin(), avail.end(), m) == avail.end()) return {};
+    if ((int)must.size() >= size)
+        return std::vector<std::string>(must.begin(), must.begin() + size);
+
+    const int need = size - (int)must.size();
+    std::map<std::pair<std::string, long>, Bucket> bmap;
+    for (const auto& d : avail) {
+        if (std::find(must.begin(), must.end(), d) != must.end()) continue;
+        auto it = locality.find(d);
+        std::pair<std::string, long> key =
+            it != locality.end() ? it->second : std::make_pair(std::string(), -1L);
+        auto& b = bmap[key];
+        b.hive = key.first;
+        b.numa = key.second;
+        b.ids.push_back(d);
+    }
+    std::vector<Bucket> buckets;
+    for (auto& kv : bmap) {
+        std::sort(kv.second.ids.begin(), kv.second.ids.end(),
+                  [](const std::string& a, const std::string& b) {
+                      return a.size() != b.size() ? a.size() < b.size() : a < b;
+                  });
+        buckets.push_back(std::move(kv.second));
+    }
+    std::sort(buckets.begin(), buckets.end(), [](const Bucket& a, const Bucket& b) {
+        if (a.ids.size() != b.ids.size()) return a.ids.size() > b.ids.size();
+        if (a.numa != b.numa) return a.numa < b.numa;
+        return a.hive < b.hive;
+    });
+
+    const int nb = (int)buckets.size();
+    std::vector<int64_t> affinity(nb, 0);
+    for (int i = 0; i < nb; i++) {
+        for (const auto& m : must) {
+            auto it = locality.find(m);
+            std::string mh = it != locality.end() ? it->second.first : "";
+            long mn = it != locality.end() ? it->second.second : -1;
+            if (!buckets[i].hive.empty() && mh == buckets[i].hive)
+                affinity[i] += W_XGMI;
+            else if (mn == buckets[i].numa && buckets[i].numa != -1)
+                affinity[i] += W_NUMA;
+        }
+    }
+    std::vector<int> caps(nb), suffix(nb + 1, 0);
+    for (int i = 0; i < nb; i++) caps[i] = (int)buckets[i].ids.size();
+    for (int i = nb - 1; i >= 0; i--) suffix[i] = suffix[i + 1] + caps[i];
+
+    std::map<std::string, int> hive_span;
+    for (int i = 0; i < nb; i++)
+        if (!buckets[i].hive.empty()) hive_span[buckets[i].hive] += caps[i];
+    std::vector<char> equiv(nb, 0);
+    for (int i = 1; i < nb; i++) {
+        const Bucket& a = buckets[i - 1];
+        const Bucket& b = buckets[i];
+        equiv[i] = !a.hive.empty() && !b.hive.empty() &&
+                   caps[i] == caps[i - 1] && a.numa == b.numa &&
+                   affinity[i] == affinity[i - 1] &&
+                   hive_span[a.hive] == caps[i - 1] &&
+                   hive_span[b.hive] == caps[i];
+    }
+
+    auto pkey = [&](int i) -> std::pair<std::string, long> {
+        if (!buckets[i].hive.empty()) return {buckets[i].hive, -1};
+        return {std::string("numa"), buckets[i].numa};
+    };
+    std::map<std::pair<std::string, long>, int> hive_free;
+    for (int i = 0; i < nb; i++) hive_free[pkey(i)] += caps[i];
+
+    std::vector<int64_t> max_aff_suffix(nb + 1, 0);
+    for (int i = nb - 1; i >= 0; i--)
+        max_aff_suffix[i] = std::max(max_aff_suffix[i + 1], affinity[i]);
+    std::vector<std::map<std::string, int>> hive_cap_suffix(nb + 1);
+    std::vector<std::map<long, int>> numa_cap_suffix(nb + 1);
+    for (int i = nb - 1; i >= 0; i--) {
+        hive_cap_suffix[i] = hive_cap_suffix[i + 1];
+        numa_cap_suffix[i] = numa_cap_suffix[i + 1];
+        if (!buckets[i].hive.empty()) hive_cap_suffix[i][buckets[i].hive] += caps[i];
+        if (buckets[i].numa != -1) numa_cap_suffix[i][buckets[i].numa] += caps[i];
+    }
+
+    std::vector<int> take(nb, 0), best_take;
+    int64_t best_score = -1;
+    int64_t best_pack = 0;
+    std::map<std::string, int> taken_hive;
+    std::map<long, int> taken_numa;
+
+    auto bucket_pair = [&](int i, int c) -> int64_t {
+        int64_t w = !buckets[i].hive.empty() ? W_XGMI
+                    : buckets[i].numa != -1 ? W_NUMA : 0;
+        return w * c * (c - 1) / 2;
+    };
+    auto packing = [&]() -> int64_t {
+        std::map<std::pair<std::string, long>, int> taken;
+        for (int i = 0; i < nb; i++)
+            if (take[i]) taken[pkey(i)] += take[i];
+        int64_t p = 0;
+        for (auto& kv : taken) p -= hive_free[kv.first] - kv.second;
+        return p;
+    };
+    auto topk_ranges = [](const std::vector<std::pair<int, int>>& ranges,
+                          int left) -> int64_t {
+        if (ranges.empty() || left <= 0) return 0;
+        int lo = 0, hi = 0;
+        for (auto& r : ranges) hi = std::max(hi, r.first + r.second);
+        while (lo < hi) {
+            int mid = (lo + hi + 1) / 2;
+            long cnt = 0;
+            for (auto& r : ranges) {
+                int top = r.first + r.second;
+                if (top > mid) cnt += top - std::max(mid, r.first);
+            }
+            if (cnt >= left) lo = mid; else hi = mid - 1;
+        }
+        const int T = lo;
+        int64_t total = 0;
+        long cnt_above = 0;
+        for (auto& r : ranges) {
+            int top = r.first + r.second;
+            int start = std::max(T + 1, r.first);
+            if (top > start) {
+                int64_t k = top - start;
+                total += k * (start + top - 1) / 2;
+                cnt_above += k;
+            }
+        }
+        total += (int64_t)(left - cnt_above) * T;
+        return total;
+    };
+    auto concentration_exact = [](const std::vector<int>& caps_desc,
+                                  int left) -> int64_t {
+        int64_t total = 0;
+        for (int cap : caps_desc) {
+            if (left <= 0) break;
+            int64_t c = cap < left ? cap : left;
+            total += c * (c - 1) / 2;
+            left -= (int)c;
+        }
+        return total;
+    };
+    std::vector<std::vector<int>> hive_caps_desc(nb + 1), numa_caps_desc(nb + 1);
+    for (int i = 0; i <= nb; i++) {
+        for (auto& kv : hive_cap_suffix[i]) hive_caps_desc[i].push_back(kv.second);
+        for (auto& kv : numa_cap_suffix[i]) numa_caps_desc[i].push_back(kv.second);
+        std::sort(hive_caps_desc[i].rbegin(), hive_caps_desc[i].rend());
+        std::sort(numa_caps_desc[i].rbegin(), numa_caps_desc[i].rend());
+    }
+    auto xgmi_upper = [&](int i, int left) -> int64_t {
+        bool untouched = true;
+        for (auto& kv : hive_cap_suffix[i]) {
+            auto it = taken_hive.find(kv.first);
+            if (it != taken_hive.end() && it->second > 0) { untouched = false; break; }
+        }
+        if (untouched) return concentration_exact(hive_caps_desc[i], left);
+        std::vector<std::pair<int, int>> ranges;
+        for (auto& kv : hive_cap_suffix[i]) {
+            auto it = taken_hive.find(kv.first);
+            int t = it != taken_hive.end() ? it->second : 0;
+            ranges.emplace_back(t, kv.second);
+        }
+        return topk_ranges(ranges, left);
+    };
+    auto numa_upper = [&](int i, int left) -> int64_t {
+        bool untouched = true;
+        for (auto& kv : numa_cap_suffix[i]) {
+            auto it = taken_numa.find(kv.first);
+            if (it != taken_numa.end() && it->second > 0) { untouched = false; break; }
+        }
+        if (untouched) return concentration_exact(numa_caps_desc[i], left);
+        std::vector<std::pair<int, int>> ranges;
+        for (auto& kv : numa_cap_suffix[i]) {
+            auto it = taken_numa.find(kv.first);
+            int t = it != taken_numa.end() ? it->second : 0;
+            ranges.emplace_back(t, kv.second);
+        }
+        return topk_ranges(ranges, left);
+    };
+
+    long nodes_visited = 0;
+    std::function<void(int, int, int64_t)> dfs = [&](int i, int left, int64_t acc) {
+        if (++nodes_visited > MAX_SEARCH_NODES && !best_take.empty()) return;
+        if (left == 0) {
+            int64_t pack = packing();
+            if (best_take.empty() || acc > best_score ||
+                (acc == best_score && pack > best_pack)) {
+                best_score = acc;
+                best_pack = pack;
+                best_take = take;
+            }
+            return;
+        }
+        if (i >= nb || suffix[i] < left) return;
+        if (!best_take.empty()) {
+            int64_t ub = acc + W_XGMI * xgmi_upper(i, left) +
+                         W_NUMA * numa_upper(i, left) +
+                         max_aff_suffix[i] * left;
+            if (ub < best_score || (ub == best_score && best_pack == 0)) return;
+        }
+        const std::string& hive = buckets[i].hive;
+        const long numa = buckets[i].numa;
+        int cmax = std::min(caps[i], left);
+        if (equiv[i]) cmax = std::min(cmax, take[i - 1]);
+        for (int c = cmax; c >= 0; c--) {
+            int64_t inc = bucket_pair(i, c) + affinity[i] * c;
+            if (c) {
+                if (!hive.empty()) inc += W_XGMI * c * taken_hive[hive];
+                if (numa != -1) inc += W_NUMA * c * taken_numa[numa];
+                take[i] = c;
+                if (!hive.empty()) taken_hive[hive] += c;
+                if (numa != -1) taken_numa[numa] += c;
+            }
+            dfs(i + 1, left - c, acc + inc);
+            if (c) {
+                take[i] = 0;
+                if (!hive.empty()) taken_hive[hive] -= c;
+                if (numa != -1) taken_numa[numa] -= c;
+            }
+        }
+    };
+    dfs(0, need, 0);
+    if (best_take.empty() && need > 0) return {};
+
+    std::vector<std::string> chosen = must;
+    for (int i = 0; i < nb; i++)
+        for (int c = 0; c < best_take[i]; c++) chosen.push_back(buckets[i].ids[c]);
+    return chosen;
+}
+
+}
+}
diff --git a/native/xpu_grpc_server.cpp b/native/xpu_grpc_server.cpp
--- a/native/xpu_grpc_server.cpp
+++ b/native/xpu_grpc_server.cpp
@@ -1,6 +1,7 @@
 #include <pybind11/pybind11.h>
 #include <pybind11/stl.h>
 
+#include <array>
 #include <atomic>
 #include <cerrno>
 #include <chrono>
@@ -21,6 +22,7 @@
 
 #include "h2.h"
 #include "pbwire.h"
+#include "prefer.h"
 
 namespace py = pybind11;
 using namespace kxdp;
@@ -34,6 +36,7 @@
 
 struct DeviceEntry {
     std::vector<std::string> bdfs;
+    std::vector<std::array<std::string, 3>> attr_paths;
     bool healthy = true;
     std::string cdi_device;
     std::string ann_key, ann_value;
@@ -41,6 +44,11 @@
 };
 
 using Table = std::unordered_map<std::string, DeviceEntry>;
+
+struct Snapshot {
+    Table table;
+    prefer::Locality locality;
+};
 
 struct AllocateConfig {
     bool enabled = false;
@@ -52,7 +60,7 @@
     bool timing = false;
 };
 
-enum class Kind { CONSTANT, WATCH, PYTHON, ALLOCATE };
+enum class Kind { CONSTANT, WATCH, PYTHON, ALLOCATE, PREFERRED };
 
 struct Method {
     Kind kind;
@@ -69,8 +77,8 @@
     return std::string(slash ? slash + 1 : buf);
 }
 
-long read_vendor(int dirfd) {
-    int fd = ::openat(dirfd, "vendor", O_RDONLY | O_CLOEXEC);
+long read_vendor(int dirfd, const char* name) {
+    int fd = ::openat(dirfd, name, O_RDONLY | O_CLOEXEC);
     if (fd < 0) return -1;
     char buf[64];
     ssize_t n = ::read(fd, buf, sizeof(buf) - 1);
@@ -148,22 +156,33 @@
         methods_[path] = Method{Kind::ALLOCATE, {}, py::object()};
     }
 
+    void configure_preferred(const std::string& path, bool timing) {
+        check_not_running();
+        preferred_timing_ = timing;
+        methods_[path] = Method{Kind::PREFERRED, {}, py::object()};
+    }
+
     void update_table(const std::vector<std::tuple<
             std::string, std::vector<std::string>, bool, py::bytes,
-            std::string, std::string, std::string>>& devices) {
-        auto t = std::make_shared<Table>();
+            std::string, std::string, std::string, std::string, long>>&
+                          devices) {
+        auto t = std::make_shared<Snapshot>();
         for (auto& d : devices) {
             DeviceEntry e;
             e.bdfs = std::get<1>(d);
+            for (const auto& bdf : e.bdfs)
+                e.attr_paths.push_back({bdf + "/iommu_group", bdf + "/vendor",
+                                        bdf + "/driver"});
             e.healthy = std::get<2>(d);
             e.cdi_device = std::string(std::get<3>(d));
             e.ann_key = std::get<4>(d);
             e.ann_value = std::get<5>(d);
             e.dev_path = std::get<6>(d);
-            (*t)[std::get<0>(d)] = std::move(e);
+            t->table[std::get<0>(d)] = std::move(e);
+            t->locality[std::get<0>(d)] = {std::get<7>(d), std::get<8>(d)};
         }
         std::lock_guard<std::mutex> g(table_mu_);
-        table_ = std::move(t);
+        snapshot_ = std::move(t);
     }
 
     void publish(const std::string& message) {
@@ -226,6 +245,11 @@
     std::vector<double> allocate_timing_us() {
         std::lock_guard<std::mutex> g(stat_mu_);
         return alloc_us_;
+    }
+
+    std::vector<double> preferred_timing_us() {
+        std::lock_guard<std::mutex> g(stat_mu_);
+        return preferred_us_;
     }
 
     void on_rpc(h2::Conn& c, uint32_t sid, const std::string& path,
@@ -239,6 +263,8 @@
             return c.reply_unary(sid, m.bytes);
         case Kind::ALLOCATE:
             return handle_allocate(c, sid, msg);
+        case Kind::PREFERRED:
+            return handle_preferred(c, sid, msg);
         case Kind::WATCH: {
             std::shared_ptr<const std::string> latest;
             {
@@ -379,8 +405,21 @@
         return dirfd_ >= 0;
     }
 
+    bool function_ok_fast(const std::string& gid,
+                          const std::array<std::string, 3>& names) {
+        if (link_base(dirfd_, names[0].c_str()) != gid) return false;
+        long vendor = read_vendor(dirfd_, names[1].c_str());
+        if (vendor < 0 ||
+            std::find(alloc_.vendors.begin(), alloc_.vendors.end(), vendor) ==
+                alloc_.vendors.end())
+            return false;
+        return link_base(dirfd_, names[2].c_str()) == alloc_.required_driver;
+    }
+
     std::string revalidate(const std::string& gid, const DeviceEntry& dev) {
-        for (const auto& bdf : dev.bdfs) {
+        for (size_t f = 0; f < dev.bdfs.size(); f++) {
+            const std::string& bdf = dev.bdfs[f];
+            if (function_ok_fast(gid, dev.attr_paths[f])) continue;
             const int flags = O_RDONLY | O_DIRECTORY | O_CLOEXEC;
             int dfd = ::openat(dirfd_, bdf.c_str(), flags);
             if (dfd < 0) {
@@ -393,7 +432,7 @@
             if (link_base(dfd, "iommu_group") != gid) {
                 err = "device " + bdf + " no longer in IOMMU group " + gid;
             } else {
-                long vendor = read_vendor(dfd);
+                long vendor = read_vendor(dfd, "vendor");
                 if (vendor < 0 ||
                     std::find(alloc_.vendors.begin(), alloc_.vendors.end(),
                               vendor) == alloc_.vendors.end())
@@ -466,17 +505,17 @@
 
     void handle_allocate(h2::Conn& c, uint32_t sid, const std::string& msg) {
         auto t0 = std::chrono::steady_clock::now();
-        std::shared_ptr<const Table> table;
+        std::shared_ptr<const Snapshot> snap;
         {
             std::lock_guard<std::mutex> g(table_mu_);
-            table = table_;
+            snap = snapshot_;
         }
         std::vector<std::vector<std::string>> reqs;
         if (!pb::parse_allocate_request(msg, reqs))
             return c.reply_error(sid, h2::GRPC_INTERNAL,
                                  "Exception deserializing request!");
         static const Table kEmpty;
-        const Table& tbl = table ? *table : kEmpty;
+        const Table& tbl = snap ? snap->table : kEmpty;
         std::string resp, err;
         for (const auto& ids : reqs) {
             std::string cresp;
@@ -502,6 +541,39 @@
             total_s_ += dt;
             if (alloc_.timing && alloc_us_.size() < kMaxTimingSamples)
                 alloc_us_.push_back(dt * 1e6);
+        }
+        c.reply_unary(sid, resp);
+    }
+
+    void handle_preferred(h2::Conn& c, uint32_t sid, const std::string& msg) {
+        auto t0 = std::chrono::steady_clock::now();
+        std::shared_ptr<const Snapshot> snap;
+        {
+            std::lock_guard<std::mutex> g(table_mu_);
+            snap = snapshot_;
+        }
+        std::vector<pb::PreferredRequest> reqs;
+        if (!pb::parse_preferred_request(msg, reqs))
+            return c.reply_error(sid, h2::GRPC_INTERNAL,
+                                 "Exception deserializing request!");
+        static const Snapshot kEmpty;
+        const Snapshot& s = snap ? *snap : kEmpty;
+        std::string resp;
+        std::vector<std::string> available;
+        for (const auto& req : reqs) {
+            available.clear();
+            for (const auto& id : req.available)
+                if (s.table.count(id)) available.push_back(id);
+            pb::put_preferred_response(
+                resp, prefer::select_preferred(s.locality, available,
+                                               req.must_include, req.size));
+        }
+        if (preferred_timing_) {
+            double dt = std::chrono::duration<double>(
+                            std::chrono::steady_clock::now() - t0).count();
+            std::lock_guard<std::mutex> g(stat_mu_);
+            if (preferred_us_.size() < kMaxTimingSamples)
+                preferred_us_.push_back(dt * 1e6);
         }
         c.reply_unary(sid, resp);
     }
@@ -669,7 +741,7 @@
     py::object on_reject_, on_watch_change_;
 
     std::mutex table_mu_;
-    std::shared_ptr<const Table> table_;
+    std::shared_ptr<const Snapshot> snapshot_;
     std::mutex pub_mu_;
     std::shared_ptr<const std::string> latest_;
     uint64_t pub_gen_ = 0;
@@ -678,7 +750,8 @@
     std::mutex stat_mu_;
     uint64_t allocations_ = 0, failures_ = 0;
     double last_s_ = 0.0, total_s_ = 0.0;
-    std::vector<double> alloc_us_;
+    std::vector<double> alloc_us_, preferred_us_;
+    bool preferred_timing_ = false;
 
     std::thread thread_;
     std::atomic<bool> stop_{false};
@@ -710,11 +783,14 @@
              py::arg("devices_dir"), py::arg("vendors"),
              py::arg("required_driver"), py::arg("on_reject"),
              py::arg("timing") = false)
+        .def("configure_preferred", &GrpcServer::configure_preferred,
+             py::arg("path"), py::arg("timing") = false)
         .def("update_table", &GrpcServer::update_table, py::arg("devices"))
         .def("publish", &GrpcServer::publish, py::arg("message"))
         .def("start", &GrpcServer::start)
         .def("stop", &GrpcServer::stop, py::arg("grace") = 1.0)
         .def("stats", &GrpcServer::stats)
         .def("allocate_timing_us", &GrpcServer::allocate_timing_us)
+        .def("preferred_timing_us", &GrpcServer::preferred_timing_us)
         .def_property_readonly("running", &GrpcServer::running);
 }
diff --git a/native/xpu_native.cpp b/native/xpu_native.cpp
--- a/native/xpu_native.cpp
+++ b/native/xpu_native.cpp
@@ -13,6 +13,8 @@
 #include <string>
 #include <unistd.h>
 #include <vector>
+
+#include "prefer.h"
 
 namespace py = pybind11;
 
@@ -203,257 +205,12 @@
     return err;
 }
 
-
-constexpr int64_t W_XGMI = 1000000000000LL;
-constexpr int64_t W_NUMA = 1000000;
-constexpr long MAX_SEARCH_NODES = 50000;
-
-struct Bucket {
-    std::string hive;
-    long numa;
-    std::vector<std::string> ids;
-};
-
 std::vector<std::string> select_preferred(
-    const std::map<std::string, std::pair<std::string, long>>& locality,
+    const kxdp::prefer::Locality& locality,
     const std::vector<std::string>& available,
     const std::vector<std::string>& must_include,
     int size) {
-    std::vector<std::string> avail;
-    for (const auto& d : available)
-        if (std::find(avail.begin(), avail.end(), d) == avail.end())
-            avail.push_back(d);
-    std::vector<std::string> must;
-    for (const auto& d : must_include)
-        if (std::find(must.begin(), must.end(), d) == must.end())
-            must.push_back(d);
-    if (size <= 0 || (size_t)size > avail.size()) return {};
-    for (const auto& m : must)
-        if (std::find(avail.begin(), avail.end(), m) == avail.end()) return {};
-    if ((int)must.size() >= size)
-        return std::vector<std::string>(must.begin(), must.begin() + size);
-
-    const int need = size - (int)must.size();
-    std::map<std::pair<std::string, long>, Bucket> bmap;
-    for (const auto& d : avail) {
-        if (std::find(must.begin(), must.end(), d) != must.end()) continue;
-        auto it = locality.find(d);
-        std::pair<std::string, long> key =
-            it != locality.end() ? it->second : std::make_pair(std::string(), -1L);
-        auto& b = bmap[key];
-        b.hive = key.first;
-        b.numa = key.second;
-        b.ids.push_back(d);
-    }
-    std::vector<Bucket> buckets;
-    for (auto& kv : bmap) {
-        std::sort(kv.second.ids.begin(), kv.second.ids.end(),
-                  [](const std::string& a, const std::string& b) {
-                      return a.size() != b.size() ? a.size() < b.size() : a < b;
-                  });
-        buckets.push_back(std::move(kv.second));
-    }
-    std::sort(buckets.begin(), buckets.end(), [](const Bucket& a, const Bucket& b) {
-        if (a.ids.size() != b.ids.size()) return a.ids.size() > b.ids.size();
-        if (a.numa != b.numa) return a.numa < b.numa;
-        return a.hive < b.hive;
-    });
-
-    const int nb = (int)buckets.size();
-    std::vector<int64_t> affinity(nb, 0);
-    for (int i = 0; i < nb; i++) {
-        for (const auto& m : must) {
-            auto it = locality.find(m);
-            std::string mh = it != locality.end() ? it->second.first : "";
-            long mn = it != locality.end() ? it->second.second : -1;
-            if (!buckets[i].hive.empty() && mh == buckets[i].hive)
-                affinity[i] += W_XGMI;
-            else if (mn == buckets[i].numa && buckets[i].numa != -1)
-                affinity[i] += W_NUMA;
-        }
-    }
-    std::vector<int> caps(nb), suffix(nb + 1, 0);
-    for (int i = 0; i < nb; i++) caps[i] = (int)buckets[i].ids.size();
-    for (int i = nb - 1; i >= 0; i--) suffix[i] = suffix[i + 1] + caps[i];
-
-    std::map<std::string, int> hive_span;
-    for (int i = 0; i < nb; i++)
-        if (!buckets[i].hive.empty()) hive_span[buckets[i].hive] += caps[i];
-    std::vector<char> equiv(nb, 0);
-    for (int i = 1; i < nb; i++) {
-        const Bucket& a = buckets[i - 1];
-        const Bucket& b = buckets[i];
-        equiv[i] = !a.hive.empty() && !b.hive.empty() &&
-                   caps[i] == caps[i - 1] && a.numa == b.numa &&
-                   affinity[i] == affinity[i - 1] &&
-                   hive_span[a.hive] == caps[i - 1] &&
-                   hive_span[b.hive] == caps[i];
-    }
-
-    auto pkey = [&](int i) -> std::pair<std::string, long> {
-        if (!buckets[i].hive.empty()) return {buckets[i].hive, -1};
-        return {std::string("numa"), buckets[i].numa};
-    };
-    std::map<std::pair<std::string, long>, int> hive_free;
-    for (int i = 0; i < nb; i++) hive_free[pkey(i)] += caps[i];
-
-    std::vector<int64_t> max_aff_suffix(nb + 1, 0);
-    for (int i = nb - 1; i >= 0; i--)
-        max_aff_suffix[i] = std::max(max_aff_suffix[i + 1], affinity[i]);
-    std::vector<std::map<std::string, int>> hive_cap_suffix(nb + 1);
-    std::vector<std::map<long, int>> numa_cap_suffix(nb + 1);
-    for (int i = nb - 1; i >= 0; i--) {
-        hive_cap_suffix[i] = hive_cap_suffix[i + 1];
-        numa_cap_suffix[i] = numa_cap_suffix[i + 1];
-        if (!buckets[i].hive.empty()) hive_cap_suffix[i][buckets[i].hive] += caps[i];
-        if (buckets[i].numa != -1) numa_cap_suffix[i][buckets[i].numa] += caps[i];
-    }
-
-    std::vector<int> take(nb, 0), best_take;
-    int64_t best_score = -1;
-    int64_t best_pack = 0;
-    std::map<std::string, int> taken_hive;
-    std::map<long, int> taken_numa;
-
-    auto bucket_pair = [&](int i, int c) -> int64_t {
-        int64_t w = !buckets[i].hive.empty() ? W_XGMI
-                    : buckets[i].numa != -1 ? W_NUMA : 0;
-        return w * c * (c - 1) / 2;
-    };
-    auto packing = [&]() -> int64_t {
-        std::map<std::pair<std::string, long>, int> taken;
-        for (int i = 0; i < nb; i++)
-            if (take[i]) taken[pkey(i)] += take[i];
-        int64_t p = 0;
-        for (auto& kv : taken) p -= hive_free[kv.first] - kv.second;
-        return p;
-    };
-    auto topk_ranges = [](const std::vector<std::pair<int, int>>& ranges,
-                          int left) -> int64_t {
-        if (ranges.empty() || left <= 0) return 0;
-        int lo = 0, hi = 0;
-        for (auto& r : ranges) hi = std::max(hi, r.first + r.second);
-        while (lo < hi) {
-            int mid = (lo + hi + 1) / 2;
-            long cnt = 0;
-            for (auto& r : ranges) {
-                int top = r.first + r.second;
-                if (top > mid) cnt += top - std::max(mid, r.first);
-            }
-            if (cnt >= left) lo = mid; else hi = mid - 1;
-        }
-        const int T = lo;
-        int64_t total = 0;
-        long cnt_above = 0;
-        for (auto& r : ranges) {
-            int top = r.first + r.second;
-            int start = std::max(T + 1, r.first);
-            if (top > start) {
-                int64_t k = top - start;
-                total += k * (start + top - 1) / 2;
-                cnt_above += k;
-            }
-        }
-        total += (int64_t)(left - cnt_above) * T;
-        return total;
-    };
-    auto concentration_exact = [](const std::vector<int>& caps_desc,
-                                  int left) -> int64_t {
-        int64_t total = 0;
-        for (int cap : caps_desc) {
-            if (left <= 0) break;
-            int64_t c = cap < left ? cap : left;
-            total += c * (c - 1) / 2;
-            left -= (int)c;
-        }
-        return total;
-    };
-    std::vector<std::vector<int>> hive_caps_desc(nb + 1), numa_caps_desc(nb + 1);
-    for (int i = 0; i <= nb; i++) {
-        for (auto& kv : hive_cap_suffix[i]) hive_caps_desc[i].push_back(kv.second);
-        for (auto& kv : numa_cap_suffix[i]) numa_caps_desc[i].push_back(kv.second);
-        std::sort(hive_caps_desc[i].rbegin(), hive_caps_desc[i].rend());
-        std::sort(numa_caps_desc[i].rbegin(), numa_caps_desc[i].rend());
-    }
-    auto xgmi_upper = [&](int i, int left) -> int64_t {
-        bool untouched = true;
-        for (auto& kv : hive_cap_suffix[i]) {
-            auto it = taken_hive.find(kv.first);
-            if (it != taken_hive.end() && it->second > 0) { untouched = false; break; }
-        }
-        if (untouched) return concentration_exact(hive_caps_desc[i], left);
-        std::vector<std::pair<int, int>> ranges;
-        for (auto& kv : hive_cap_suffix[i]) {
-            auto it = taken_hive.find(kv.first);
-            int t = it != taken_hive.end() ? it->second : 0;
-            ranges.emplace_back(t, kv.second);
-        }
-        return topk_ranges(ranges, left);
-    };
-    auto numa_upper = [&](int i, int left) -> int64_t {
-        bool untouched = true;
-        for (auto& kv : numa_cap_suffix[i]) {
-            auto it = taken_numa.find(kv.first);
-            if (it != taken_numa.end() && it->second > 0) { untouched = false; break; }
-        }
-        if (untouched) return concentration_exact(numa_caps_desc[i], left);
-        std::vector<std::pair<int, int>> ranges;
-        for (auto& kv : numa_cap_suffix[i]) {
-            auto it = taken_numa.find(kv.first);
-            int t = it != taken_numa.end() ? it->second : 0;
-            ranges.emplace_back(t, kv.second);
-        }
-        return topk_ranges(ranges, left);
-    };
-
-    long nodes_visited = 0;
-    std::function<void(int, int, int64_t)> dfs = [&](int i, int left, int64_t acc) {
-        if (++nodes_visited > MAX_SEARCH_NODES && !best_take.empty()) return;
-        if (left == 0) {
-            int64_t pack = packing();
-            if (best_take.empty() || acc > best_score ||
-                (acc == best_score && pack > best_pack)) {
-                best_score = acc;
-                best_pack = pack;
-                best_take = take;
-            }
-            return;
-        }
-        if (i >= nb || suffix[i] < left) return;
-        if (!best_take.empty()) {
-            int64_t ub = acc + W_XGMI * xgmi_upper(i, left) +
-                         W_NUMA * numa_upper(i, left) +
-                         max_aff_suffix[i] * left;
-            if (ub < best_score || (ub == best_score && best_pack == 0)) return;
-        }
-        const std::string& hive = buckets[i].hive;
-        const long numa = buckets[i].numa;
-        int cmax = std::min(caps[i], left);
-        if (equiv[i]) cmax = std::min(cmax, take[i - 1]);
-        for (int c = cmax; c >= 0; c--) {
-            int64_t inc = bucket_pair(i, c) + affinity[i] * c;
-            if (c) {
-                if (!hive.empty()) inc += W_XGMI * c * taken_hive[hive];
-                if (numa != -1) inc += W_NUMA * c * taken_numa[numa];
-                take[i] = c;
-                if (!hive.empty()) taken_hive[hive] += c;
-                if (numa != -1) taken_numa[numa] += c;
-            }
-            dfs(i + 1, left - c, acc + inc);
-            if (c) {
-                take[i] = 0;
-                if (!hive.empty()) taken_hive[hive] -= c;
-                if (numa != -1) taken_numa[numa] -= c;
-            }
-        }
-    };
-    dfs(0, need, 0);
-    if (best_take.empty() && need > 0) return {};
-
-    std::vector<std::string> chosen = must;
-    for (int i = 0; i < nb; i++)
-        for (int c = 0; c < best_take[i]; c++) chosen.push_back(buckets[i].ids[c]);
-    return chosen;
+    return kxdp::prefer::select_preferred(locality, available, must_include, size);
 }
 
 }
diff --git a/setup.py b/setup.py
--- a/setup.py
+++ b/setup.py
@@ -66,7 +66,7 @@
                     sources=["native/xpu_native.cpp",
                              "native/xpu_grpc_server.cpp"],
                     depends=["native/h2.h", "native/hpack.h",
-                             "native/pbwire.h"],
+                             "native/pbwire.h", "native/prefer.h"],
                     include_dirs=[pybind11.get_include(), "native"],
                     extra_compile_args=["-O2", "-std=c++17"],
                     extra_link_args=["-pthread"],
```

New measurement: 52.34 us. +7.2%, slower.
